# Daniel-Starr/pointcloudhookup

Measured on AMD Instinct MI355X. Metric: Mpts/s ground-filter+tower-cluster, 100 M-pt corridor; % HBM roofline on kNN, higher is better.
Workload: dtype f32 (filter) + f64 (distance predicate)

## Files before the change

pointcloudhookup_amd/csrc/pch_common.h:

```cpp
#pragma once
#include <hip/hip_runtime.h>
#include <stdint.h>
#include <stddef.h>
#include <stdio.h>
#include <string.h>

#include "../../include/pch_hip.h"

namespace pch {

void set_error(const char* fmt, ...);

#define PCH_HIP_TRY(expr)                                                         \
    do {                                                                          \
        hipError_t _e = (expr);                                                   \
        if (_e != hipSuccess) {                                                   \
            ::pch::set_error("%s failed: %s (%s:%d)", #expr, hipGetErrorString(_e), \
                             __FILE__, __LINE__);                                 \
            return PCH_ERR_HIP;                                                   \
        }                                                                         \
    } while (0)

#define PCH_TRY(expr)                  \
    do {                               \
        int _rc = (expr);              \
        if (_rc != PCH_OK) return _rc; \
    } while (0)

#define PCH_REQUIRE(cond, msg)                                   \
    do {                                                         \
        if (!(cond)) {                                           \
            ::pch::set_error("%s: %s", __func__, msg);           \
            return PCH_ERR_ARG;                                  \
        }                                                        \
    } while (0)

constexpr int PCH_MAX_DEVICES = 16;
struct DeviceGuard {
    int rc, prev, dev;
    explicit DeviceGuard(const void* device_ptr);
    ~DeviceGuard();
    DeviceGuard(const DeviceGuard&) = delete;
    DeviceGuard& operator=(const DeviceGuard&) = delete;
};
int current_device_slot();
bool may_release_hip_objects();
#define PCH_DEVICE_GUARD(ptr)                 \
    ::pch::DeviceGuard _pch_guard(ptr);       \
    if (_pch_guard.rc != PCH_OK) return _pch_guard.rc

void ws_touched(const void* base, size_t bytes);
struct Arena {
    char*  base;
    size_t cap;
    size_t off;
    bool   overflow;
    explicit Arena(void* b = nullptr, size_t c = 0, bool continues = false)
        : base(static_cast<char*>(b)), cap(c), off(0), overflow(false) {
        if (b && !continues) ws_touched(b, c);
    }
    template <typename T>
    T* take(size_t count) {
        size_t bytes = (count * sizeof(T) + 255) & ~size_t(255);
        size_t at = off;
        off += bytes;
        if (!base) return nullptr;
        if (off > cap) { overflow = true; return nullptr; }
        return reinterpret_cast<T*>(base + at);
    }
    size_t mark() const { return off; }
    void   reset(size_t m) { off = m; }
};

struct HostPeek {
    void*      pinned;
    hipEvent_t ev;
    bool       ok;
};
HostPeek& host_peek();
int peek_enqueue(const void* dev, size_t bytes, hipStream_t s);
int peek_wait(void* dst, size_t bytes);

struct DbBoxOut { uint32_t* acc; int32_t cap; bool done; };
struct GfEarly { const void* dev; size_t bytes; };
int ground_filter_run(const float* raw, int64_t n, double pct, float offset, float fallback_offset, int64_t min_keep,
                      float* out_points, int32_t* out_index, float* out_scalars, int64_t* out_count, float* out_aabb,
                      void* ws, size_t ws_bytes, hipStream_t s, const GfEarly* early);
int dbscan_run(const float* xyz, int64_t n, double eps, int32_t min_samples, int64_t chunk_size,
               const float* aabb_host, int32_t* labels, uint8_t* core, int32_t* out_nclusters,
               void* ws, size_t ws_bytes, hipStream_t s, int32_t* k_host, DbBoxOut* box = nullptr);
int segment_run(const int32_t* labels, const float* xyz, int64_t n, int32_t nclusters, int32_t* out_perm,
                int64_t* out_offsets, float* out_stats, void* ws, size_t ws_bytes, hipStream_t s, bool stats_encoded);

bool prof_enabled();
bool prof_wanted(const char* name);
void prof_pre(const char* name, hipStream_t s);
void prof_post(hipStream_t s);

#define PCH_LAUNCH(name, kernel, grid, block, shmem, stream, ...)                  \
    do {                                                                           \
        const bool _prof = ::pch::prof_enabled() && ::pch::prof_wanted(name);            \
        if (_prof) ::pch::prof_pre(name, stream);                                  \
        hipLaunchKernelGGL(kernel, grid, block, shmem, stream, __VA_ARGS__);       \
        if (_prof) ::pch::prof_post(stream);                                       \
        hipError_t _le = hipGetLastError();                                        \
        if (_le != hipSuccess) {                                                   \
            ::pch::set_error("launch %s failed: %s", name, hipGetErrorString(_le)); \
            return PCH_ERR_HIP;                                                    \
        }                                                                          \
    } while (0)

static inline int64_t ceil_div(int64_t a, int64_t b) { return (a + b - 1) / b; }
static inline int bits_for(uint64_t count) {
    int b = 0;
    while (b < 64 && (uint64_t(1) << b) < count) ++b;
    return b;
}

#ifdef __HIPCC__
constexpr int WAVE = 64;

__device__ __forceinline__ int lane_id() { return threadIdx.x & 63; }
__device__ __forceinline__ int wave_id() { return threadIdx.x >> 6; }

__device__ __forceinline__ uint32_t f32_ordered(float f) {
    uint32_t u = __float_as_uint(f);
    return (u & 0x80000000u) ? ~u : (u | 0x80000000u);
}
__device__ __forceinline__ float f32_unordered(uint32_t k) {
    uint32_t u = (k & 0x80000000u) ? (k & 0x7fffffffu) : ~k;
    return __uint_as_float(u);
}
__device__ __forceinline__ uint64_t f64_ordered(double d) {
    uint64_t u = (uint64_t)__double_as_longlong(d);
    return (u & 0x8000000000000000ull) ? ~u : (u | 0x8000000000000000ull);
}
__device__ __forceinline__ double f64_unordered(uint64_t k) {
    uint64_t u = (k & 0x8000000000000000ull) ? (k & 0x7fffffffffffffffull) : ~k;
    return __longlong_as_double((long long)u);
}

__device__ __forceinline__ uint64_t lanemask_lt() {
    return (uint64_t(1) << lane_id()) - 1;
}

template <typename T>
__device__ __forceinline__ T wave_reduce_add(T v) {
#pragma unroll
    for (int o = 32; o > 0; o >>= 1) v += __shfl_xor(v, o, 64);
    return v;
}
template <typename T>
__device__ __forceinline__ T wave_reduce_min(T v) {
#pragma unroll
    for (int o = 32; o > 0; o >>= 1) { T w = __shfl_xor(v, o, 64); v = w < v ? w : v; }
    return v;
}
template <typename T>
__device__ __forceinline__ T wave_reduce_max(T v) {
#pragma unroll
    for (int o = 32; o > 0; o >>= 1) { T w = __shfl_xor(v, o, 64); v = w > v ? w : v; }
    return v;
}
template <typename T>
__device__ __forceinline__ T wave_scan_incl(T v) {
    const int l = lane_id();
#pragma unroll
    for (int o = 1; o < 64; o <<= 1) { T w = __shfl_up(v, o, 64); if (l >= o) v += w; }
    return v;
}
template <int BITS>
__device__ __forceinline__ uint32_t wave_match(uint32_t d, bool valid, uint32_t& peers_out) {
    uint32_t nlo = 0, nhi = 0;
#pragma unroll
    for (int b = 0; b < BITS; ++b) {
        const int32_t B = ((int32_t)(d << (31 - b))) >> 31;
        const uint64_t m = __ballot(B != 0);
        nlo |= (uint32_t)m ^ (uint32_t)B;
        nhi |= (uint32_t)(m >> 32) ^ (uint32_t)B;
    }
    const uint64_t v = __ballot(valid);
    const uint32_t plo = (uint32_t)v & ~nlo, phi = (uint32_t)(v >> 32) & ~nhi;
    peers_out = (uint32_t)__popc(plo) + (uint32_t)__popc(phi);
    return __builtin_amdgcn_mbcnt_hi(phi, __builtin_amdgcn_mbcnt_lo(plo, 0u));
}
#endif

}
```

pointcloudhookup_amd/csrc/pch_dbscan.hip:

```cpp
#include "pch_prims.h"

namespace pch {

constexpr int DB_THREADS = 256;
constexpr int DB_WAVES   = DB_THREADS / 64;
constexpr int DB_ROWS    = 25;
constexpr int INT_BIG    = 0x7fffffff;
constexpr int DB_FEW_QUERIES = 24;
constexpr int DB_AHEAD = 3;
constexpr long long DB_LONG_TOT = 8192;
constexpr int DB_SEGS = 43;

struct DbGrid {
    float   ox, oy, oz;
    double  cell;
    double  inv_cell;
    double  eps2;
    float   eps2_lo, eps2_hi;
    int     bx, by, bz;
    int     mx, my, mz;
    int64_t chunk_size;
    const uint32_t* chunk_bad;
    const uint32_t* chunk_cells;
    int     min_samples;
};

__constant__ int8_t DB_ROW_DY[DB_ROWS] = {0, 1, -1, 0, 0, 1, 1, -1, -1, 2, -2, 0, 0,
                                          2, 2, -2, -2, 1, 1, -1, -1, 2, 2, -2, -2};
__constant__ int8_t DB_ROW_DZ[DB_ROWS] = {0, 0, 0, 1, -1, 1, -1, 1, -1, 0, 0, 2, -2,
                                          1, -1, 1, -1, 2, -2, 2, -2, 2, -2, 2, -2};

__device__ __forceinline__ uint64_t db_pack(const DbGrid& g, uint64_t chunk, uint64_t cz,
                                            uint64_t cy, uint64_t cx) {
    return ((((chunk << g.bz) | cz) << g.by | cy) << g.bx) | cx;
}

__device__ __forceinline__ bool db_within(const float4& q, const float4& p, double eps2) {
    const double dx = (double)q.x - (double)p.x;
    const double dy = (double)q.y - (double)p.y;
    const double dz = (double)q.z - (double)p.z;
    double d = dx * dx;
    d += dy * dy;
    d += dz * dz;
    return d <= eps2;
}

__device__ __forceinline__ bool db_within2(const float4& q, const float4& p, const DbGrid& g) {
    const float dx = q.x - p.x, dy = q.y - p.y, dz = q.z - p.z;
    float d = dx * dx;
    d = __builtin_fmaf(dy, dy, d);
    d = __builtin_fmaf(dz, dz, d);
    if (d <= g.eps2_lo) return true;
    if (d >= g.eps2_hi) return false;
    return db_within(q, p, g.eps2);
}

typedef float f32x2 __attribute__((ext_vector_type(2)));
struct __attribute__((aligned(16))) DbPair { f32x2 x, y, z, pad; };

__device__ __forceinline__ void db_tile_put(DbPair* __restrict__ tile, int l, const float4& p) {
    float* f = reinterpret_cast<float*>(&tile[l >> 1]);
    f[l & 1] = p.x; f[2 + (l & 1)] = p.y; f[4 + (l & 1)] = p.z;
}
__device__ __forceinline__ float4 db_tile_get(const DbPair* __restrict__ tile, int k) {
    const float* f = reinterpret_cast<const float*>(&tile[k >> 1]);
    float4 p;
    p.x = f[k & 1]; p.y = f[2 + (k & 1)]; p.z = f[4 + (k & 1)]; p.w = 0.0f;
    return p;
}
__device__ __forceinline__ int db_tile_count(const float4& q, const DbPair* __restrict__ tile, int nj,
                                             const DbGrid& g) {
    const f32x2 qx = {q.x, q.x}, qy = {q.y, q.y}, qz = {q.z, q.z};
    const float lo = g.eps2_lo, hi = g.eps2_hi;
    int c_lo = 0, c_hi = 0;
    const int np = ((nj + 7) & ~7) >> 1;
    for (int k = 0; k < np; k += 4) {
        f32x2 px[4], py[4], pz[4];
#pragma unroll
        for (int u = 0; u < 4; ++u) { px[u] = tile[k + u].x; py[u] = tile[k + u].y; pz[u] = tile[k + u].z; }
#pragma unroll
        for (int u = 0; u < 4; ++u) {
            const f32x2 dx = qx - px[u], dy = qy - py[u], dz = qz - pz[u];
            f32x2 d = dx * dx;
            d = __builtin_elementwise_fma(dy, dy, d);
            d = __builtin_elementwise_fma(dz, dz, d);
            c_lo += (d.x <= lo ? 1 : 0) + (d.y <= lo ? 1 : 0);
            c_hi += (d.x < hi ? 1 : 0) + (d.y < hi ? 1 : 0);
        }
    }
    if (c_lo != c_hi) {
        c_lo = 0;
        for (int k = 0; k < nj; ++k) c_lo += db_within2(q, db_tile_get(tile, k), g) ? 1 : 0;
    }
    return c_lo;
}

__device__ __forceinline__ double db_box_d2(const float4& q, const float* __restrict__ box) {
    const double gx = fmax(fmax((double)box[0] - (double)q.x, (double)q.x - (double)box[3]), 0.0);
    const double gy = fmax(fmax((double)box[1] - (double)q.y, (double)q.y - (double)box[4]), 0.0);
    const double gz = fmax(fmax((double)box[2] - (double)q.z, (double)q.z - (double)box[5]), 0.0);
    double d = gx * gx;
    d += gy * gy;
    d += gz * gz;
    return d;
}
__device__ __forceinline__ double db_boxbox_d2(const float* __restrict__ a, const float* __restrict__ b) {
    const double gx = fmax(fmax((double)b[0] - (double)a[3], (double)a[0] - (double)b[3]), 0.0);
    const double gy = fmax(fmax((double)b[1] - (double)a[4], (double)a[1] - (double)b[4]), 0.0);
    const double gz = fmax(fmax((double)b[2] - (double)a[5], (double)a[2] - (double)b[5]), 0.0);
    double d = gx * gx;
    d += gy * gy;
    d += gz * gz;
    return d;
}

__device__ __forceinline__ bool db_row_bad(const float* __restrict__ xyz, int64_t i) {
    const uint32_t a = __float_as_uint(xyz[3 * i + 0]) & 0x7FFFFFFFu;
    const uint32_t b = __float_as_uint(xyz[3 * i + 1]) & 0x7FFFFFFFu;
    const uint32_t c = __float_as_uint(xyz[3 * i + 2]) & 0x7FFFFFFFu;
    return a >= 0x7F800000u || b >= 0x7F800000u || c >= 0x7F800000u;
}
__global__ __launch_bounds__(DB_THREADS) void db_chunkbad_k(const float* __restrict__ xyz, int64_t n,
                                                            int64_t chunk_size, uint32_t* __restrict__ bad) {
    for (int64_t i = (int64_t)blockIdx.x * DB_THREADS + threadIdx.x; i < n;
         i += (int64_t)gridDim.x * DB_THREADS)
        if (db_row_bad(xyz, i)) atomicOr(&bad[i / chunk_size], 1u);
}

__global__ __launch_bounds__(DB_THREADS) void db_first_bad_k(const float* __restrict__ xyz, int64_t n,
                                                             unsigned long long* __restrict__ first) {
    unsigned long long best = ~0ull;
    for (int64_t i = (int64_t)blockIdx.x * DB_THREADS + threadIdx.x; i < n;
         i += (int64_t)gridDim.x * DB_THREADS)
        if (db_row_bad(xyz, i) && (unsigned long long)i < best) best = (unsigned long long)i;
    best = wave_reduce_min(best);
    if (lane_id() == 0 && best != ~0ull) atomicMin(first, best);
}

__global__ __launch_bounds__(DB_THREADS) void db_aabb_in_k(const float* __restrict__ xyz, int64_t n,
                                                           uint32_t* __restrict__ mm) {
    uint32_t lo[3] = {0xFFFFFFFFu, 0xFFFFFFFFu, 0xFFFFFFFFu}, hi[3] = {0u, 0u, 0u};
    for (int64_t i = (int64_t)blockIdx.x * DB_THREADS + threadIdx.x; i < n;
         i += (int64_t)gridDim.x * DB_THREADS) {
        const float x = xyz[3 * i + 0], y = xyz[3 * i + 1], z = xyz[3 * i + 2];
        if (!(fabsf(x) < INFINITY && fabsf(y) < INFINITY && fabsf(z) < INFINITY)) continue;
        const float v[3] = {x, y, z};
#pragma unroll
        for (int a = 0; a < 3; ++a) {
            const uint32_t k = f32_ordered(v[a]);
            lo[a] = k < lo[a] ? k : lo[a];
            hi[a] = k > hi[a] ? k : hi[a];
        }
    }
#pragma unroll
    for (int a = 0; a < 3; ++a) {
        lo[a] = wave_reduce_min(lo[a]);
        hi[a] = wave_reduce_max(hi[a]);
        if (lane_id() == 0) {
            if (lo[a] != 0xFFFFFFFFu) atomicMin(&mm[a], lo[a]);
            if (hi[a] != 0u) atomicMax(&mm[3 + a], hi[a]);
        }
    }
}

__device__ __forceinline__ bool db_cell_coords(const DbGrid& g, float x, float y, float z,
                                               uint32_t& cx, uint32_t& cy, uint32_t& cz) {
    const double fx = floor(((double)x - (double)g.ox) * g.inv_cell);
    const double fy = floor(((double)y - (double)g.oy) * g.inv_cell);
    const double fz = floor(((double)z - (double)g.oz) * g.inv_cell);
    const bool ok = fx >= 0.0 && fx <= (double)g.mx && fy >= 0.0 && fy <= (double)g.my &&
                    fz >= 0.0 && fz <= (double)g.mz;
    cx = ok ? (uint32_t)fx : 0u; cy = ok ? (uint32_t)fy : 0u; cz = ok ? (uint32_t)fz : 0u;
    return ok;
}

__global__ __launch_bounds__(DB_THREADS) void db_keys_k(const float* __restrict__ xyz, int64_t n,
                                                        DbGrid g, const uint32_t* __restrict__ bad,
                                                        uint64_t* __restrict__ keys,
                                                        uint32_t* __restrict__ vals,
                                                        uint32_t* __restrict__ status) {
    const int64_t i = (int64_t)blockIdx.x * DB_THREADS + threadIdx.x;
    if (i >= n) return;
    vals[i] = (uint32_t)i;
    if (bad[i / g.chunk_size]) {
        keys[i] = db_pack(g, (uint64_t)(i / g.chunk_size), 0, 0, 0);
        return;
    }
    const float x = xyz[3 * i + 0], y = xyz[3 * i + 1], z = xyz[3 * i + 2];
    uint32_t cx, cy, cz;
    if (!db_cell_coords(g, x, y, z, cx, cy, cz)) atomicOr(status, 1u);
    keys[i] = db_pack(g, (uint64_t)(i / g.chunk_size), cz, cy, cx);
}

__global__ __launch_bounds__(DB_THREADS) void dbc_axis_keys_k(const float* __restrict__ xyz, int64_t n, int axis,
                                                              uint64_t* __restrict__ keys, uint32_t* __restrict__ vals) {
    const int64_t i = (int64_t)blockIdx.x * DB_THREADS + threadIdx.x;
    if (i >= n) return;
    keys[i] = f32_ordered(xyz[3 * i + axis]);
    vals[i] = (uint32_t)i;
}
__global__ __launch_bounds__(DB_THREADS) void dbc_heads_k(const uint64_t* __restrict__ keys, int64_t n, double inv_cell,
                                                          uint32_t* __restrict__ head) {
    const int64_t i = (int64_t)blockIdx.x * DB_THREADS + threadIdx.x;
    if (i >= n) return;
    bool h = i == 0;
    if (i > 0) {
        const double a = (double)f32_unordered((uint32_t)keys[i - 1]), b = (double)f32_unordered((uint32_t)keys[i]);
        h = (b - a) * inv_cell >= 3.0;
    }
    head[i] = h ? 1u : 0u;
}
__global__ __launch_bounds__(DB_THREADS) void dbc_local_k(const uint64_t* __restrict__ keys, const uint32_t* __restrict__ flag,
                                                          const uint32_t* __restrict__ excl, int64_t n, double inv_cell,
                                                          float* __restrict__ headx, int phase,
                                                          uint32_t* __restrict__ li, uint32_t* __restrict__ seglen,
                                                          uint32_t* __restrict__ status) {
    const int64_t i = (int64_t)blockIdx.x * DB_THREADS + threadIdx.x;
    if (i >= n) return;
    const uint32_t seg = excl[i] + flag[i] - 1u;
    const float x = f32_unordered((uint32_t)keys[i]);
    if (phase == 0) {
        if (flag[i]) headx[seg] = x;
        return;
    }
    const double v = floor(((double)x - (double)headx[seg]) * inv_cell);
    uint32_t u = 0;
    if (v >= 0.0 && v < 2147483000.0) u = (uint32_t)v; else atomicOr(status, 2u);
    li[i] = u;
    const bool last = i + 1 == n || flag[i + 1] != 0u;
    if (last) seglen[seg] = u + 3u;
}
__global__ __launch_bounds__(DB_THREADS) void dbc_comp_k(const uint32_t* __restrict__ vals, const uint32_t* __restrict__ flag,
                                                         const uint32_t* __restrict__ excl, const uint32_t* __restrict__ li,
                                                         const uint32_t* __restrict__ segoff, int64_t n, int axis,
                                                         uint32_t* __restrict__ comp, uint32_t* __restrict__ cmax) {
    const int64_t i = (int64_t)blockIdx.x * DB_THREADS + threadIdx.x;
    if (i >= n) return;
    const uint32_t seg = excl[i] + flag[i] - 1u;
    const uint32_t c = segoff[seg] + li[i];
    comp[3 * (int64_t)vals[i] + axis] = c;
    if (i == n - 1) cmax[axis] = c;
}
__global__ __launch_bounds__(DB_THREADS) void db_keys_comp_k(const uint32_t* __restrict__ comp, int64_t n, DbGrid g,
                                                             uint64_t* __restrict__ keys, uint32_t* __restrict__ vals) {
    const int64_t i = (int64_t)blockIdx.x * DB_THREADS + threadIdx.x;
    if (i >= n) return;
    vals[i] = (uint32_t)i;
    keys[i] = db_pack(g, 0, comp[3 * i + 2], comp[3 * i + 1], comp[3 * i + 0]);
}
__global__ __launch_bounds__(DB_THREADS) void db_add_offset_k(int32_t* __restrict__ labels, int64_t n, int32_t off) {
    const int64_t i = (int64_t)blockIdx.x * DB_THREADS + threadIdx.x;
    if (i < n && labels[i] >= 0) labels[i] += off;
}

__global__ __launch_bounds__(DB_THREADS) void db_gather_k(const float* __restrict__ xyz,
                                                          const uint64_t* __restrict__ keys,
                                                          const uint32_t* __restrict__ vals, int64_t n,
                                                          float4* __restrict__ pts) {
    const int64_t i = (int64_t)blockIdx.x * DB_THREADS + threadIdx.x;
    if (i >= n) return;
    const uint32_t o = vals[i];
    float4 p;
    p.x = xyz[3 * (int64_t)o + 0];
    p.y = xyz[3 * (int64_t)o + 1];
    p.z = xyz[3 * (int64_t)o + 2];
    p.w = __uint_as_float(o);
    pts[i] = p;
}

struct Row3 { float x, y, z; };
constexpr int CS_THREADS = 1024;
constexpr int CS_WAVES   = CS_THREADS / 64;
constexpr int CS_ROUNDS  = 4;
constexpr int CS_TILE    = CS_THREADS * CS_ROUNDS;
constexpr int CS_PASSES  = 4;
constexpr int CS_HREP    = 4;
constexpr int CS_BINS    = 512;
constexpr int64_t CS_MAX_CHUNK = 1 << 17;
constexpr int64_t CS_MIN_CHUNKS = 96;

__device__ __forceinline__ uint32_t cs_cell_key(const DbGrid& g, float x, float y, float z, bool& ok) {
    uint32_t cx, cy, cz;
    ok = db_cell_coords(g, x, y, z, cx, cy, cz);
    return (((cz << g.by) | cy) << g.bx) | cx;
}

__global__ __launch_bounds__(CS_THREADS) void db_chunksort_k(
    const float* __restrict__ xyz, int64_t n, DbGrid g, const uint32_t* __restrict__ gate, uint32_t* __restrict__ bad,
    float4* __restrict__ xbuf, float4* __restrict__ pts, uint64_t* __restrict__ keys_out,
    uint32_t* __restrict__ status, unsigned long long* __restrict__ stamps) {
    if (gate[blockIdx.x] == 0u) return;
#ifdef PCH_CS_STAMPS
    int stamp_i = 0;
#define CS_STAMP() if (stamps && blockIdx.x == gridDim.x / 2 && threadIdx.x == 0) stamps[stamp_i++] = wall_clock64();
    unsigned long long tacc[3] = {0, 0, 0}, tlast = 0;
#define CS_TILE_STAMP(k) do { const unsigned long long _t = wall_clock64(); tacc[k] += _t - tlast; tlast = _t; } while (0)
#else
#define CS_STAMP()
#define CS_TILE_STAMP(k)
#endif
    CS_STAMP();
    __shared__ uint32_t hist[CS_PASSES][CS_HREP][CS_BINS];
    __shared__ uint32_t cnt[CS_WAVES][CS_BINS];
    __shared__ uint32_t off[CS_WAVES][CS_BINS];
    __shared__ uint32_t base[CS_BINS];
    __shared__ uint32_t wsum[CS_BINS / 64];
    __shared__ uint32_t flags[2];
    __shared__ uint32_t cbox[6];
    const int tid = threadIdx.x, w = wave_id(), l = lane_id();
    const int64_t c = blockIdx.x;
    const int64_t lo = c * g.chunk_size;
    const int cn = (int)((n - lo) < g.chunk_size ? (n - lo) : g.chunk_size);
    const Row3* __restrict__ rows = reinterpret_cast<const Row3*>(xyz) + lo;
    for (int j = tid; j < CS_PASSES * CS_HREP * CS_BINS; j += CS_THREADS) (&hist[0][0][0])[j] = 0;
    for (int j = tid; j < CS_WAVES * CS_BINS; j += CS_THREADS) (&cnt[0][0])[j] = 0;
    if (tid < 2) flags[tid] = 0;
    if (tid < 6) cbox[tid] = tid < 3 ? 0xFFFFFFFFu : 0u;
    __syncthreads();
    constexpr int HU = 8;
    {
        uint32_t mn[3] = {0xFFFFFFFFu, 0xFFFFFFFFu, 0xFFFFFFFFu}, mx[3] = {0u, 0u, 0u};
        for (int i0 = 0; i0 < cn; i0 += HU * CS_THREADS) {
            Row3 q[HU];
#pragma unroll
            for (int u = 0; u < HU; ++u) {
                const int i = i0 + u * CS_THREADS + tid;
                q[u] = rows[i < cn ? i : 0];
            }
#pragma unroll
            for (int u = 0; u < HU; ++u) {
                const bool in = i0 + u * CS_THREADS + tid < cn;
                const bool fin = fabsf(q[u].x) < INFINITY && fabsf(q[u].y) < INFINITY && fabsf(q[u].z) < INFINITY;
                uint32_t cc[3];
                const bool ok = db_cell_coords(g, q[u].x, q[u].y, q[u].z, cc[0], cc[1], cc[2]);
                if (in && !fin) flags[0] = 1u;
                else if (in && !ok) flags[1] = 1u;
                if (in && fin && ok) {
#pragma unroll
                    for (int a = 0; a < 3; ++a) { mn[a] = cc[a] < mn[a] ? cc[a] : mn[a]; mx[a] = cc[a] > mx[a] ? cc[a] : mx[a]; }
                }
            }
        }
#pragma unroll
        for (int a = 0; a < 3; ++a) {
            const uint32_t lo_w = wave_reduce_min(mn[a]), hi_w = wave_reduce_max(mx[a]);
            if (l == 0) { atomicMin(&cbox[a], lo_w); atomicMax(&cbox[3 + a], hi_w); }
        }
    }
    __syncthreads();
    CS_STAMP();
    const uint32_t ox = cbox[0], oy = cbox[1], oz = cbox[2];
    const bool any = cbox[3] >= ox && cbox[4] >= oy && cbox[5] >= oz;
    const int wx = any && cbox[3] > ox ? 32 - __clz(cbox[3] - ox) : 0;
    const int wy = any && cbox[4] > oy ? 32 - __clz(cbox[4] - oy) : 0;
    const int wz = any && cbox[5] > oz ? 32 - __clz(cbox[5] - oz) : 0;
    const int tb = wx + wy + wz;
    const int passes = (tb + 8) / 9;
    const int dbits = passes ? (tb + passes - 1) / passes : 1;
    const uint32_t mask = (1u << dbits) - 1u;
    const uint32_t gxm = (1u << g.bx) - 1u, gym = (1u << g.by) - 1u;
    auto relkey = [&](uint32_t k) -> uint32_t {
        const uint32_t cx = k & gxm, cy = (k >> g.bx) & gym, cz = k >> (g.bx + g.by);
        return (uint32_t)((((((uint64_t)(cz - oz)) << wy) | (uint64_t)(cy - oy)) << wx) | (uint64_t)(cx - ox));
    };
    for (int i0 = 0; i0 < cn; i0 += HU * CS_THREADS) {
        Row3 q[HU];
#pragma unroll
        for (int u = 0; u < HU; ++u) {
            const int i = i0 + u * CS_THREADS + tid;
            q[u] = rows[i < cn ? i : 0];
        }
#pragma unroll
        for (int u = 0; u < HU; ++u) {
            const bool in = i0 + u * CS_THREADS + tid < cn;
            bool ok;
            const uint32_t k = relkey(cs_cell_key(g, q[u].x, q[u].y, q[u].z, ok));
            if (in)
                for (int p = 0; p < passes; ++p) atomicAdd(&hist[p][l & (CS_HREP - 1)][(k >> (p * dbits)) & mask], 1u);
        }
    }
    __syncthreads();
    const bool isbad = flags[0] != 0;
    CS_STAMP();
    if (tid == 0) {
        bad[c] = isbad ? 1u : 0u;
        if (!isbad && flags[1]) atomicOr(status, 1u);
    }
    const int sh = g.bx + g.by + g.bz;
    const uint64_t hi = sh < 64 ? ((uint64_t)c << sh) : 0ull;
    if (isbad || passes == 0) {
        for (int i = tid; i < cn; i += CS_THREADS) {
            const Row3 q = rows[i];
            float4 o4;
            o4.x = q.x; o4.y = q.y; o4.z = q.z; o4.w = __uint_as_float((uint32_t)(lo + i));
            pts[lo + i] = o4;
            bool ok;
            keys_out[lo + i] = isbad ? hi : (hi | cs_cell_key(g, q.x, q.y, q.z, ok));
        }
        return;
    }
    auto run_pass = [&](int p, auto FIRST_T, auto LAST_T) {
        constexpr bool FIRST = decltype(FIRST_T)::value, LAST = decltype(LAST_T)::value;
        const int shift = p * dbits;
        const float4* __restrict__ src = ((passes - p) & 1) ? xbuf + lo : pts + lo;
        float4* __restrict__ dst = ((passes - 1 - p) & 1) ? xbuf + lo : pts + lo;
        uint32_t hv = 0, incl = 0;
        if (tid < CS_BINS) {
            hv = 0;
#pragma unroll
            for (int r = 0; r < CS_HREP; ++r) hv += hist[p][r][tid];
            incl = wave_scan_incl(hv);
            if (l == 63) wsum[w] = incl;
        }
        __syncthreads();
        if (tid < CS_BINS) {
            uint32_t b = incl - hv;
            for (int w2 = 0; w2 < w; ++w2) b += wsum[w2];
            base[tid] = b;
        }
        __syncthreads();
        auto fetch = [&](int t0, float4 (&out)[CS_ROUNDS]) {
            const int seg = t0 + w * (64 * CS_ROUNDS);
#pragma unroll
            for (int r = 0; r < CS_ROUNDS; ++r) {
                const int i = seg + r * 64 + l;
                const int j = i < cn ? i : 0;
                if constexpr (FIRST) {
                    const Row3 q = rows[j];
                    out[r].x = q.x; out[r].y = q.y; out[r].z = q.z;
                    out[r].w = __uint_as_float((uint32_t)(lo + j));
                } else {
                    out[r] = src[j];
                }
            }
        };
        float4 nxt[CS_ROUNDS];
        auto tile = [&](int t0, auto FULL_T) {
            constexpr bool FULL = decltype(FULL_T)::value;
            float4 row[CS_ROUNDS];
            uint32_t key[CS_ROUNDS], rank[CS_ROUNDS];
            const int seg = t0 + w * (64 * CS_ROUNDS);
#pragma unroll
            for (int r = 0; r < CS_ROUNDS; ++r) row[r] = nxt[r];
            if (t0 + CS_TILE < cn) fetch(t0 + CS_TILE, nxt);
#ifdef PCH_CS_STAMPS
            tlast = wall_clock64();
#endif
#pragma unroll
            for (int r = 0; r < CS_ROUNDS; ++r) {
                const bool valid = FULL || seg + r * 64 + l < cn;
                bool ok;
                key[r] = cs_cell_key(g, row[r].x, row[r].y, row[r].z, ok);
                const uint32_t d = (relkey(key[r]) >> shift) & mask;
                uint32_t np;
                const uint32_t rk = dbits <= 8 ? wave_match<8>(d, valid, np) : wave_match<9>(d, valid, np);
                const uint32_t prior = cnt[w][d];
                __builtin_amdgcn_wave_barrier();
                if (valid && rk == 0) cnt[w][d] = prior + np;
                __builtin_amdgcn_wave_barrier();
                rank[r] = prior + rk;
            }
            __syncthreads();
            CS_TILE_STAMP(0);
            if (tid < CS_BINS) {
                uint32_t run = base[tid];
#pragma unroll
                for (int w2 = 0; w2 < CS_WAVES; ++w2) {
                    const uint32_t cc = cnt[w2][tid];
                    off[w2][tid] = run;
                    cnt[w2][tid] = 0;
                    run += cc;
                }
                base[tid] = run;
            }
            __syncthreads();
            CS_TILE_STAMP(1);
#pragma unroll
            for (int r = 0; r < CS_ROUNDS; ++r) {
                if (FULL || seg + r * 64 + l < cn) {
                    const uint32_t d = (relkey(key[r]) >> shift) & mask;
                    const uint32_t pos = off[w][d] + rank[r];
                    dst[pos] = row[r];
                    if constexpr (LAST) keys_out[lo + pos] = hi | key[r];
                }
            }
            CS_TILE_STAMP(2);
        };
        fetch(0, nxt);
        int t0 = 0;
        for (; t0 + CS_TILE <= cn; t0 += CS_TILE) tile(t0, std::true_type{});
        if (t0 < cn) tile(t0, std::false_type{});
        __syncthreads();
        CS_STAMP();
    };
    for (int p = 0; p < passes; ++p) {
        const bool first = p == 0, last = p == passes - 1;
        if (first && last) run_pass(p, std::true_type{}, std::true_type{});
        else if (first)    run_pass(p, std::true_type{}, std::false_type{});
        else if (last)     run_pass(p, std::false_type{}, std::true_type{});
        else               run_pass(p, std::false_type{}, std::false_type{});
    }
#ifdef PCH_CS_STAMPS
    __syncthreads();
    CS_STAMP();
    if (stamps && blockIdx.x == gridDim.x / 2 && threadIdx.x == 0) for (int k = 0; k < 3; ++k) stamps[8 + k] = tacc[k];
#endif
}

constexpr int CT_SLOTS = 4096;
constexpr int CT_BITS  = 12;
constexpr int CT_CELLS = 1024;
constexpr uint32_t CT_EMPTY = 0xFFFFFFFFu;
static_assert(CT_SLOTS == 1 << CT_BITS && CT_CELLS + CS_THREADS < CT_SLOTS, "the table never fills (see sweep 1)");

__device__ __forceinline__ uint32_t ct_hash(uint32_t k) { return (k * 0x9E3779B1u) >> (32 - CT_BITS); }

__global__ __launch_bounds__(CS_THREADS) void db_cellscatter_k(
    const float* __restrict__ xyz, int64_t n, DbGrid g, uint32_t* __restrict__ bad, uint32_t* __restrict__ ovf,
    float4* __restrict__ pts, uint64_t* __restrict__ keys_out, uint32_t* __restrict__ status) {
    __shared__ uint32_t tkey[CT_SLOTS];
    __shared__ uint32_t tcnt[CT_SLOTS];
    __shared__ uint32_t skey[CT_CELLS];
    __shared__ uint32_t wsum[CS_WAVES];
    __shared__ uint32_t flags[5];
    const int tid = threadIdx.x, w = wave_id(), l = lane_id();
    const int64_t c = blockIdx.x;
    const int64_t lo = c * g.chunk_size;
    const int cn = (int)((n - lo) < g.chunk_size ? (n - lo) : g.chunk_size);
    const Row3* __restrict__ rows = reinterpret_cast<const Row3*>(xyz) + lo;
    for (int j = tid; j < CT_SLOTS; j += CS_THREADS) { tkey[j] = CT_EMPTY; tcnt[j] = 0u; }
    if (tid < 5) flags[tid] = 0u;
    __syncthreads();
    constexpr int HU = 8;
    for (int i0 = 0; i0 < cn; i0 += HU * CS_THREADS) {
        if (__hip_atomic_load(&flags[3], __ATOMIC_RELAXED, __HIP_MEMORY_SCOPE_WORKGROUP)) break;
        Row3 q[HU];
#pragma unroll
        for (int u = 0; u < HU; ++u) {
            const int i = i0 + u * CS_THREADS + tid;
            q[u] = rows[i < cn ? i : 0];
        }
#pragma unroll
        for (int u = 0; u < HU; ++u) {
            const bool in = i0 + u * CS_THREADS + tid < cn;
            const bool fin = fabsf(q[u].x) < INFINITY && fabsf(q[u].y) < INFINITY && fabsf(q[u].z) < INFINITY;
            bool ok;
            const uint32_t k = cs_cell_key(g, q[u].x, q[u].y, q[u].z, ok);
            if (in && !fin) flags[0] = 1u;
            else if (in && !ok) flags[1] = 1u;
            if (in && fin && __hip_atomic_load(&flags[3], __ATOMIC_RELAXED, __HIP_MEMORY_SCOPE_WORKGROUP) == 0u) {
                uint32_t h = ct_hash(k);
                for (int p = 0; p < CT_SLOTS; ++p, h = (h + 1u) & (CT_SLOTS - 1)) {
                    const uint32_t old = atomicCAS(&tkey[h], CT_EMPTY, k);
                    if (old == CT_EMPTY && atomicAdd(&flags[2], 1u) >= (uint32_t)CT_CELLS) flags[3] = 1u;
                    if (old == CT_EMPTY || old == k) { atomicAdd(&tcnt[h], 1u); break; }
                }
            }
        }
    }
    __syncthreads();
    const bool isbad = flags[0] != 0u;
    const uint32_t ncell = flags[2];
    const bool over = !isbad && ncell > (uint32_t)CT_CELLS;
    if (tid == 0) {
        ovf[c] = over ? 1u : 0u;
        if (!over) {
            bad[c] = isbad ? 1u : 0u;
            if (!isbad && flags[1]) atomicOr(status, 1u);
        }
    }
    if (over) return;
    const int sh = g.bx + g.by + g.bz;
    const uint64_t hi = sh < 64 ? ((uint64_t)c << sh) : 0ull;
    if (isbad || ncell == 1u) {
        for (int i = tid; i < cn; i += CS_THREADS) {
            const Row3 q = rows[i];
            float4 o4;
            o4.x = q.x; o4.y = q.y; o4.z = q.z; o4.w = __uint_as_float((uint32_t)(lo + i));
            pts[lo + i] = o4;
            bool ok;
            keys_out[lo + i] = isbad ? hi : (hi | cs_cell_key(g, q.x, q.y, q.z, ok));
        }
        return;
    }
    const int P = 1 << (32 - __clz((int)ncell - 1));
    for (int j0 = 0; j0 < CT_SLOTS; j0 += CS_THREADS) {
        const uint32_t k = tkey[j0 + tid];
        const uint64_t m = __ballot(k != CT_EMPTY);
        uint32_t base = 0;
        if (l == 0 && m) base = atomicAdd(&flags[4], (uint32_t)__popcll(m));
        base = (uint32_t)__shfl((int)base, 0, 64);
        if (k != CT_EMPTY) skey[base + (uint32_t)__popcll(m & lanemask_lt())] = k;
    }
    for (int j = (int)ncell + tid; j < P; j += CS_THREADS) skey[j] = CT_EMPTY;
    __syncthreads();
    for (int k = 2; k <= P; k <<= 1) {
        for (int j = k >> 1; j > 0; j >>= 1) {
            for (int t = tid; t < P / 2; t += CS_THREADS) {
                const int a = 2 * t - (t & (j - 1)), b = a + j;
                const uint32_t ka = skey[a], kb = skey[b];
                if ((ka > kb) == ((a & k) == 0)) { skey[a] = kb; skey[b] = ka; }
            }
            __syncthreads();
        }
    }
    {
        uint32_t slot[4], cnt[4], sum = 0;
#pragma unroll
        for (int u = 0; u < 4; ++u) {
            const int j = 4 * tid + u;
            slot[u] = 0; cnt[u] = 0;
            if (j < (int)ncell) {
                const uint32_t k = skey[j];
                uint32_t h = ct_hash(k);
                for (int p = 0; p < CT_SLOTS && tkey[h] != k; ++p) h = (h + 1u) & (CT_SLOTS - 1);
                slot[u] = h;
                cnt[u] = tcnt[h];
            }
            sum += cnt[u];
        }
        const uint32_t incl = wave_scan_incl(sum);
        if (l == 63) wsum[w] = incl;
        __syncthreads();
        uint32_t run = incl - sum;
        for (int w2 = 0; w2 < w; ++w2) run += wsum[w2];
#pragma unroll
        for (int u = 0; u < 4; ++u) {
            if (4 * tid + u < (int)ncell) tcnt[slot[u]] = run;
            run += cnt[u];
        }
    }
    __syncthreads();
    for (int i0 = 0; i0 < cn; i0 += HU * CS_THREADS) {
        Row3 q[HU];
#pragma unroll
        for (int u = 0; u < HU; ++u) {
            const int i = i0 + u * CS_THREADS + tid;
            q[u] = rows[i < cn ? i : 0];
        }
#pragma unroll
        for (int u = 0; u < HU; ++u) {
            const int i = i0 + u * CS_THREADS + tid;
            if (i < cn) {
                bool ok;
                const uint32_t k = cs_cell_key(g, q[u].x, q[u].y, q[u].z, ok);
                uint32_t h = ct_hash(k);
                for (int p = 0; p < CT_SLOTS && tkey[h] != k; ++p) h = (h + 1u) & (CT_SLOTS - 1);
                const uint32_t pos = atomicAdd(&tcnt[h], 1u);
                if (pos >= (uint32_t)cn) continue;
                float4 o4;
                o4.x = q[u].x; o4.y = q[u].y; o4.z = q[u].z; o4.w = __uint_as_float((uint32_t)(lo + i));
                pts[lo + pos] = o4;
                keys_out[lo + pos] = hi | k;
            }
        }
    }
}

constexpr int DC_ITEMS = SCAN_TILE / DB_THREADS;
static_assert(DC_ITEMS == 8, "two 64-byte key loads per thread");

__device__ __forceinline__ void dc_load_keys(const uint64_t* __restrict__ keys, int64_t base, int64_t n,
                                             uint64_t (&k)[DC_ITEMS], uint64_t& prev) {
    if (base + DC_ITEMS <= n) {
        const ulonglong2* q = reinterpret_cast<const ulonglong2*>(keys + base);
#pragma unroll
        for (int j = 0; j < DC_ITEMS / 2; ++j) { const ulonglong2 v = q[j]; k[2 * j] = v.x; k[2 * j + 1] = v.y; }
    } else {
#pragma unroll
        for (int j = 0; j < DC_ITEMS; ++j) k[j] = base + j < n ? keys[base + j] : 0ull;
    }
    prev = (base > 0 && base < n) ? keys[base - 1] : 0ull;
}

__global__ __launch_bounds__(DB_THREADS) void db_heads_k(const uint64_t* __restrict__ keys, int64_t n,
                                                         uint32_t* __restrict__ tile_sums) {
    __shared__ uint32_t wsum[DB_WAVES];
    const int64_t base = (int64_t)blockIdx.x * SCAN_TILE + (int64_t)threadIdx.x * DC_ITEMS;
    uint64_t k[DC_ITEMS], prev;
    dc_load_keys(keys, base, n, k, prev);
    uint32_t heads = 0;
#pragma unroll
    for (int j = 0; j < DC_ITEMS; ++j) {
        const int64_t i = base + j;
        heads += (i < n && (i == 0 || k[j] != (j ? k[j - 1] : prev))) ? 1u : 0u;
    }
    heads = wave_reduce_add(heads);
    if (lane_id() == 0) wsum[wave_id()] = heads;
    __syncthreads();
    if (threadIdx.x == 0) {
        uint32_t t = 0;
#pragma unroll
        for (int w = 0; w < DB_WAVES; ++w) t += wsum[w];
        tile_sums[blockIdx.x] = t;
    }
}

__global__ __launch_bounds__(DB_THREADS) void db_cells_k(const uint64_t* __restrict__ keys,
                                                         const uint32_t* __restrict__ tile_excl, int64_t n,
                                                         int sh, int64_t nchunks,
                                                         uint32_t* __restrict__ cid,
                                                         uint32_t* __restrict__ cell_start,
                                                         uint64_t* __restrict__ cell_key,
                                                         uint32_t* __restrict__ chunk_cells,
                                                         uint32_t* __restrict__ cell_acc) {
    __shared__ uint32_t wsum[DB_WAVES];
    const int64_t base = (int64_t)blockIdx.x * SCAN_TILE + (int64_t)threadIdx.x * DC_ITEMS;
    uint64_t k[DC_ITEMS], prev;
    dc_load_keys(keys, base, n, k, prev);
    bool hd[DC_ITEMS];
    uint32_t heads = 0;
#pragma unroll
    for (int j = 0; j < DC_ITEMS; ++j) {
        const int64_t i = base + j;
        hd[j] = i < n && (i == 0 || k[j] != (j ? k[j - 1] : prev));
        heads += hd[j] ? 1u : 0u;
    }
    const uint32_t incl = wave_scan_incl(heads);
    if (lane_id() == 63) wsum[wave_id()] = incl;
    __syncthreads();
    uint32_t c = tile_excl[blockIdx.x] + incl - heads;
    for (int w = 0; w < wave_id(); ++w) c += wsum[w];
    uint32_t cc[DC_ITEMS];
#pragma unroll
    for (int j = 0; j < DC_ITEMS; ++j) {
        const int64_t i = base + j;
        c += hd[j] ? 1u : 0u;
        cc[j] = c - 1u;
        if (hd[j]) {
            const uint64_t key = k[j], pk = j ? k[j - 1] : prev;
            cell_start[cc[j]] = (uint32_t)i;
            cell_key[cc[j]] = key;
            uint4* a4 = reinterpret_cast<uint4*>(cell_acc + 8 * (int64_t)cc[j]);
            a4[0] = make_uint4(0u, 0u, 0u, 0u);
            a4[1] = make_uint4(0u, 0u, 0u, 0u);
            const uint64_t ch = sh < 64 ? key >> sh : 0, pch = sh < 64 ? pk >> sh : 0;
            if (i == 0 || ch != pch) chunk_cells[ch] = cc[j];
        }
        if (i == n - 1) { cell_start[cc[j] + 1] = (uint32_t)n; chunk_cells[nchunks] = cc[j] + 1; }
    }
    if (base + DC_ITEMS <= n) {
        uint4* o = reinterpret_cast<uint4*>(cid + base);
        o[0] = make_uint4(cc[0], cc[1], cc[2], cc[3]);
        o[1] = make_uint4(cc[4], cc[5], cc[6], cc[7]);
    } else {
#pragma unroll
        for (int j = 0; j < DC_ITEMS; ++j)
            if (base + j < n) cid[base + j] = cc[j];
    }
}
struct RowSet {
    int ca[DB_ROWS], cb[DB_ROWS];
};

__device__ __forceinline__ int db_lower(const uint64_t* __restrict__ a, int m, uint64_t k) {
    int lo = 0, hi = m;
    while (lo < hi) { const int mid = (lo + hi) >> 1; if (a[mid] < k) lo = mid + 1; else hi = mid; }
    return lo;
}
__device__ __forceinline__ int2 db_row_run(const DbGrid& g, const uint64_t* __restrict__ cell_key, uint64_t key,
                                           int row) {
    const uint64_t cx = key & ((1ull << g.bx) - 1);
    const uint64_t cy = (key >> g.bx) & ((1ull << g.by) - 1);
    const uint64_t cz = (key >> (g.bx + g.by)) & ((1ull << g.bz) - 1);
    const int sh = g.bx + g.by + g.bz;
    const uint64_t chunk = sh < 64 ? (key >> sh) : 0;
    const int ny = (int)cy + DB_ROW_DY[row], nz = (int)cz + DB_ROW_DZ[row];
    int2 v;
    v.x = 0; v.y = 0;
    if (ny >= 0 && ny <= g.my && nz >= 0 && nz <= g.mz) {
        const int xlo = (int)cx - 2 < 0 ? 0 : (int)cx - 2;
        const int xhi = (int)cx + 2 > g.mx ? g.mx : (int)cx + 2;
        const int c0 = (int)g.chunk_cells[chunk], c1 = (int)g.chunk_cells[chunk + 1];
        v.x = c0 + db_lower(cell_key + c0, c1 - c0, db_pack(g, chunk, (uint64_t)nz, (uint64_t)ny, (uint64_t)xlo));
        const uint64_t khi = db_pack(g, chunk, (uint64_t)nz, (uint64_t)ny, (uint64_t)xhi);
        uint64_t kk[5];
#pragma unroll
        for (int i = 0; i < 5; ++i) kk[i] = v.x + i < c1 ? cell_key[v.x + i] : ~0ull;
        int cntx = 0;
#pragma unroll
        for (int i = 0; i < 5; ++i) cntx += kk[i] <= khi ? 1 : 0;
        v.y = v.x + cntx;
    }
    return v;
}

__device__ __forceinline__ void db_rows(const DbGrid& g, const uint64_t* __restrict__ cell_key, uint64_t key,
                                        RowSet* __restrict__ rs, const int2* __restrict__ rowtab, int cell) {
    const int l = lane_id();
    if (rowtab) {
        if (l < DB_ROWS) {
            const int2 v = rowtab[(int64_t)cell * DB_ROWS + l];
            rs->ca[l] = v.x;
            rs->cb[l] = v.y;
        }
        __builtin_amdgcn_wave_barrier();
        return;
    }
    if (l < DB_ROWS) {
        const int2 v = db_row_run(g, cell_key, key, l);
        rs->ca[l] = v.x;
        rs->cb[l] = v.y;
    }
    __builtin_amdgcn_wave_barrier();
}

__global__ __launch_bounds__(DB_THREADS) void db_rowtab_k(DbGrid g, const uint64_t* __restrict__ cell_key,
                                                          int m, int2* __restrict__ rowtab) {
    const int c = (blockIdx.x * DB_WAVES + wave_id()) * 2 + (lane_id() >> 5);
    const int l = lane_id() & 31;
    if (c >= m || l >= DB_ROWS) return;
    rowtab[(int64_t)c * DB_ROWS + l] = db_row_run(g, cell_key, cell_key[c], l);
}

template <bool COUNT>
__global__ __launch_bounds__(DB_THREADS) void db_core_k(DbGrid g, const float4* __restrict__ pts,
                                                        const uint32_t* __restrict__ cell_start,
                                                        const uint64_t* __restrict__ cell_key, int m,
                                                        const int2* __restrict__ rowtab,
                                                        uint8_t* __restrict__ core_s,
                                                        uint32_t* __restrict__ cell_ncore,
                                                        unsigned long long* __restrict__ stats) {
    unsigned long long n_useful = 0, n_slots = 0, n_tiles = 0;
    auto tally = [&]() {
        if (COUNT && lane_id() == 0) {
            atomicAdd(&stats[0], n_useful); atomicAdd(&stats[1], n_slots);
            atomicAdd(&stats[2], 1ull); atomicAdd(&stats[3], n_tiles);
        }
    };
    __shared__ RowSet rows[DB_WAVES];
    __shared__ DbPair tiles[DB_WAVES][32];
    __shared__ uint32_t seg_a[DB_WAVES][DB_SEGS], seg_b[DB_WAVES][DB_SEGS];
    const int c = blockIdx.x * DB_WAVES + wave_id();
    if (c >= m) return;
    const int l = lane_id();
    const uint32_t s = cell_start[c], e = cell_start[c + 1];
    const int cnt = (int)(e - s);
    {
        const int sh = g.bx + g.by + g.bz;
        if (g.chunk_bad[sh < 64 ? (cell_key[c] >> sh) : 0]) {
            for (uint32_t i = s + l; i < e; i += 64) core_s[i] = 0;
            if (l == 0) cell_ncore[c] = 0;
            return;
        }
    }
    if (cnt >= g.min_samples) {
        for (uint32_t i = s + l; i < e; i += 64) core_s[i] = 1;
        if (l == 0) cell_ncore[c] = (uint32_t)cnt;
        return;
    }
    RowSet* rs = &rows[wave_id()];
    db_rows(g, cell_key, cell_key[c], rs, rowtab, c);
    long long tot = 0;
    if (l < DB_ROWS) tot = (long long)cell_start[rs->cb[l]] - (long long)cell_start[rs->ca[l]];
    tot = wave_reduce_add(tot);
    if (tot < (long long)g.min_samples) {
        for (uint32_t i = s + l; i < e; i += 64) core_s[i] = 0;
        if (l == 0) cell_ncore[c] = 0;
        return;
    }
    uint32_t* sa = seg_a[wave_id()];
    uint32_t* sb = seg_b[wave_id()];
    {
        const uint64_t xmask = (1ull << g.bx) - 1;
        const int cx = (int)(cell_key[c] & xmask);
        if (l < DB_ROWS) {
            const int ca = rs->ca[l], cb = rs->cb[l];
            if (l < 9) {
                int ia = ca, ib = cb;
                if (ca < cb) {
                    if ((int)(cell_key[ca] & xmask) == cx - 2) ia = ca + 1;
                    if (ib > ia && (int)(cell_key[cb - 1] & xmask) == cx + 2) ib = cb - 1;
                }
                sa[l] = cell_start[ia];      sb[l] = cell_start[ib];
                sa[9 + l] = cell_start[ca];  sb[9 + l] = cell_start[ia];
                sa[18 + l] = cell_start[ib]; sb[18 + l] = cell_start[cb];
            } else {
                sa[18 + l] = cell_start[ca]; sb[18 + l] = cell_start[cb];
            }
        }
        __builtin_amdgcn_wave_barrier();
    }
    uint32_t ncore = 0;
    const bool long_sweep = tot >= DB_LONG_TOT;
    if (cnt < DB_FEW_QUERIES) {
        for (uint32_t q = s; q < e; ++q) {
            const float4 qp = pts[q];
            int count = 0;
            if (long_sweep) {
                for (int r = 0; r < DB_SEGS && count < g.min_samples; ++r) {
                    const uint32_t pa = sa[r], pb = sb[r];
                    for (uint32_t j0 = pa; j0 < pb && count < g.min_samples; j0 += 64u * DB_AHEAD) {
                        float4 P[DB_AHEAD];
#pragma unroll
                        for (int u = 0; u < DB_AHEAD; ++u) {
                            const uint32_t j = j0 + 64u * u + l;
                            P[u] = pts[j < pb ? j : pb - 1];
                        }
#pragma unroll
                        for (int u = 0; u < DB_AHEAD; ++u) {
                            const uint32_t jb = j0 + 64u * u;
                            const bool hit = jb + l < pb && db_within2(qp, P[u], g);
                            count += (int)__popcll(__ballot(hit));
                            if (COUNT && jb < pb) { n_useful += (pb - jb) < 64u ? (pb - jb) : 64u; n_slots += 64; }
                        }
                    }
                }
            } else {
                for (int r = 0; r < DB_SEGS && count < g.min_samples; ++r) {
                    const uint32_t pa = sa[r], pb = sb[r];
                    for (uint32_t j0 = pa; j0 < pb && count < g.min_samples; j0 += 64) {
                        const uint32_t j = j0 + l;
                        bool hit = false;
                        if (j < pb) hit = db_within2(qp, pts[j], g);
                        count += (int)__popcll(__ballot(hit));
                        if (COUNT) { n_useful += (pb - j0) < 64u ? (pb - j0) : 64u; n_slots += 64; }
                    }
                }
            }
            const bool is_core = count >= g.min_samples;
            if (l == 0) core_s[q] = is_core ? 1 : 0;
            ncore += is_core;
        }
        if (l == 0) cell_ncore[c] = ncore;
        tally();
        return;
    }
    DbPair* tile = tiles[wave_id()];
    for (uint32_t q0 = s; q0 < e; q0 += 64) {
        const bool valid = q0 + l < e;
        float4 Q;
        Q.x = Q.y = Q.z = 3.0e37f; Q.w = 0.0f;
        if (valid) Q = pts[q0 + l];
        int count = 0;
        unsigned long long active = __ballot(valid);
        int r = 0;
        uint32_t j0 = sa[0];
        while (r < DB_SEGS && __popcll(active) >= DB_FEW_QUERIES / 2) {
            const uint32_t pb = sb[r];
            if (j0 >= pb) { ++r; if (r < DB_SEGS) j0 = sa[r]; continue; }
            const int nj = (int)((pb - j0) < 64u ? (pb - j0) : 64u);
            float4 P;
            P.x = P.y = P.z = 3.0e38f; P.w = 0.0f;
            if (l < nj) P = pts[j0 + l];
            __builtin_amdgcn_wave_barrier();
            db_tile_put(tile, l, P);
            __builtin_amdgcn_wave_barrier();
            count += db_tile_count(Q, tile, nj, g);
            if (COUNT) {
                n_useful += (unsigned long long)__popcll(__ballot(valid)) * (unsigned)nj;
                n_slots += 64ull * (unsigned)((nj + 7) & ~7);
                ++n_tiles;
            }
            j0 += 64;
            active = __ballot(valid && count < g.min_samples);
        }
        while (active) {
            const int ql = (int)__builtin_ctzll(active);
            active &= active - 1;
            float4 qp;
            qp.x = __shfl(Q.x, ql, 64); qp.y = __shfl(Q.y, ql, 64); qp.z = __shfl(Q.z, ql, 64); qp.w = 0.0f;
            int cq = __shfl(count, ql, 64);
            int rr = r;
            uint32_t jj = j0;
            if (long_sweep) {
                while (rr < DB_SEGS && cq < g.min_samples) {
                    const uint32_t pb = sb[rr];
                    if (jj >= pb) { ++rr; if (rr < DB_SEGS) jj = sa[rr]; continue; }
                    float4 P[DB_AHEAD];
#pragma unroll
                    for (int u = 0; u < DB_AHEAD; ++u) {
                        const uint32_t j = jj + 64u * u + l;
                        P[u] = pts[j < pb ? j : pb - 1];
                    }
#pragma unroll
                    for (int u = 0; u < DB_AHEAD; ++u) {
                        const uint32_t jb = jj + 64u * u;
                        const bool hit = jb + l < pb && db_within2(qp, P[u], g);
                        cq += (int)__popcll(__ballot(hit));
                        if (COUNT && jb < pb) { n_useful += (pb - jb) < 64u ? (pb - jb) : 64u; n_slots += 64; }
                    }
                    jj += 64u * DB_AHEAD;
                }
            } else {
                while (rr < DB_SEGS && cq < g.min_samples) {
                    const uint32_t pb = sb[rr];
                    if (jj >= pb) { ++rr; if (rr < DB_SEGS) jj = sa[rr]; continue; }
                    const uint32_t j = jj + l;
                    bool hit = false;
                    if (j < pb) hit = db_within2(qp, pts[j], g);
                    cq += (int)__popcll(__ballot(hit));
                    if (COUNT) { n_useful += (pb - jj) < 64u ? (pb - jj) : 64u; n_slots += 64; }
                    jj += 64;
                }
            }
            if (l == ql) count = cq;
        }
        const bool is_core = valid && count >= g.min_samples;
        if (valid) core_s[q0 + l] = is_core ? 1 : 0;
        ncore += (uint32_t)__popcll(__ballot(is_core));
    }
    if (l == 0) cell_ncore[c] = ncore;
    tally();
}

constexpr int DB_CS_ROUNDS = 16;

__device__ __forceinline__ void db_cellstats_flush(uint32_t* __restrict__ acc, uint32_t c, const uint32_t (&v)[7]) {
#pragma unroll
    for (int k = 0; k < 7; ++k)
        if (v[k]) atomicMax(&acc[8 * (int64_t)c + k], v[k]);
}

__global__ __launch_bounds__(DB_THREADS) void db_cellstats_k(const float4* __restrict__ pts,
                                                             const uint32_t* __restrict__ cid,
                                                             const uint8_t* __restrict__ core_s, int64_t n,
                                                             uint32_t* __restrict__ acc,
                                                             uint32_t* __restrict__ bits, int64_t nw) {
    {
        const int64_t t = (int64_t)blockIdx.x * DB_THREADS + threadIdx.x;
        if (t < nw) bits[t] = 0u;
    }
    const int64_t base = ((int64_t)blockIdx.x * DB_WAVES + wave_id()) * (64 * DB_CS_ROUNDS);
    if (base >= n) return;
    const int l = lane_id();
    constexpr uint32_t NONE = 0xFFFFFFFFu;
    uint32_t carry_c = NONE;
    uint32_t carry[7] = {0, 0, 0, 0, 0, 0, 0};
    uint32_t mine[7] = {0, 0, 0, 0, 0, 0, 0};
    auto fold_mine = [&]() {
#pragma unroll
        for (int k = 0; k < 7; ++k) {
            const uint32_t t = wave_reduce_max(mine[k]);
            carry[k] = t > carry[k] ? t : carry[k];
            mine[k] = 0;
        }
    };
    for (int r0 = 0; r0 < DB_CS_ROUNDS; r0 += 4) {
    if (base + r0 * 64 >= n) break;
    uint32_t c4[4], core4[4];
    float4 p4[4];
#pragma unroll
    for (int u = 0; u < 4; ++u) {
        const int64_t i = base + (r0 + u) * 64 + l;
        const bool in = i < n;
        c4[u] = in ? cid[i] : NONE - 1u;
        core4[u] = in ? core_s[i] : 0u;
        p4[u] = pts[in ? i : base];
    }
#pragma unroll
    for (int u = 0; u < 4; ++u) {
        const int64_t i = base + (r0 + u) * 64 + l;
        const bool in = i < n;
        const uint32_t c = c4[u];
        uint32_t v[7] = {0, 0, 0, 0, 0, 0, 0};
        if (core4[u]) {
            const float4 p = p4[u];
            const uint32_t kx = f32_ordered(p.x), ky = f32_ordered(p.y), kz = f32_ordered(p.z);
            v[0] = ~kx; v[1] = ~ky; v[2] = ~kz; v[3] = kx; v[4] = ky; v[5] = kz;
            v[6] = ~__float_as_uint(p.w);
        }
        if (__ballot(c != carry_c) == 0) {
#pragma unroll
            for (int k = 0; k < 7; ++k) mine[k] = v[k] > mine[k] ? v[k] : mine[k];
            continue;
        }
        if (carry_c != NONE) fold_mine();
#pragma unroll
        for (int o = 1; o < 64; o <<= 1) {
            const uint32_t cu = __shfl_up(c, o, 64);
            const bool same = l >= o && cu == c;
#pragma unroll
            for (int k = 0; k < 7; ++k) {
                const uint32_t t = __shfl_up(v[k], o, 64);
                if (same) v[k] = t > v[k] ? t : v[k];
            }
        }
        const uint32_t c0 = (uint32_t)__builtin_amdgcn_readlane((int)c, 0);
        if (carry_c != NONE) {
            if (carry_c == c0) {
                if (c == c0) {
#pragma unroll
                    for (int k = 0; k < 7; ++k) v[k] = carry[k] > v[k] ? carry[k] : v[k];
                }
            } else if (l == 0) {
                db_cellstats_flush(acc, carry_c, carry);
            }
        }
        const uint32_t cn = __shfl_down(c, 1, 64);
        const bool run_end = l == 63 || cn != c;
        if (run_end && l != 63 && in) db_cellstats_flush(acc, c, v);
        carry_c = (uint32_t)__builtin_amdgcn_readlane((int)c, 63);
        if (carry_c == NONE - 1u) carry_c = NONE;
#pragma unroll
        for (int k = 0; k < 7; ++k) carry[k] = (uint32_t)__builtin_amdgcn_readlane((int)v[k], 63);
    }
    }
    if (carry_c != NONE) {
        fold_mine();
        if (l == 0) db_cellstats_flush(acc, carry_c, carry);
    }
}

__global__ __launch_bounds__(DB_THREADS) void db_cellfin_k(const uint32_t* __restrict__ acc, int m,
                                                           float* __restrict__ cell_box,
                                                           int* __restrict__ cell_min,
                                                           int* __restrict__ parent,
                                                           int* __restrict__ comp_min) {
    const int c = blockIdx.x * DB_THREADS + threadIdx.x;
    if (c >= m) return;
    uint32_t a[7];
#pragma unroll
    for (int k = 0; k < 7; ++k) a[k] = acc[8 * (int64_t)c + k];
    float box[6];
#pragma unroll
    for (int k = 0; k < 3; ++k) {
        box[k] = INFINITY;
        box[3 + k] = -INFINITY;
        if (a[k] != 0u) box[k] = f32_unordered(~a[k]);
        if (a[3 + k] != 0u) box[3 + k] = f32_unordered(a[3 + k]);
    }
#pragma unroll
    for (int k = 0; k < 6; ++k) cell_box[6 * (int64_t)c + k] = box[k];
    int mn = INT_BIG;
    if (a[6] != 0u) mn = (int)(~a[6]);
    cell_min[c] = mn;
    parent[c] = c;
    comp_min[c] = INT_BIG;
}

__device__ __forceinline__ float db_d2f(const float4& a, const float4& b) {
    const float dx = a.x - b.x, dy = a.y - b.y, dz = a.z - b.z;
    return __builtin_fmaf(dz, dz, __builtin_fmaf(dy, dy, dx * dx));
}
__device__ __forceinline__ float db_box_d2f(const float4& q, const float* __restrict__ box) {
    const float gx = fmaxf(fmaxf(box[0] - q.x, q.x - box[3]), 0.0f);
    const float gy = fmaxf(fmaxf(box[1] - q.y, q.y - box[4]), 0.0f);
    const float gz = fmaxf(fmaxf(box[2] - q.z, q.z - box[5]), 0.0f);
    return __builtin_fmaf(gz, gz, __builtin_fmaf(gy, gy, gx * gx));
}
template <typename F>
__device__ __forceinline__ int db_argmin(const float4* __restrict__ pts, const uint8_t* __restrict__ core_s,
                                         uint32_t s, uint32_t e, bool dense, F f) {
    const int l = lane_id();
    unsigned long long best = ~0ull;
    for (uint32_t i0 = s; i0 < e; i0 += 256) {
#pragma unroll
        for (int u = 0; u < 4; ++u) {
            const uint32_t i = i0 + 64 * u + l;
            if (i < e && (dense || core_s[i])) {
                const float d = f(pts[i]);
                const unsigned long long k = ((unsigned long long)__float_as_uint(d) << 32) | i;
                best = k < best ? k : best;
            }
        }
    }
    best = wave_reduce_min(best);
    return best == ~0ull ? -1 : (int)(uint32_t)best;
}

__device__ __forceinline__ bool db_cells_connected(const DbGrid& g, const float4* __restrict__ pts,
                                                   const uint8_t* __restrict__ core_s, uint32_t as, uint32_t ae,
                                                   bool a_dense, uint32_t bs, uint32_t be, bool b_dense,
                                                   const float* __restrict__ boxB, uint32_t a_from) {
    const int l = lane_id();
    if (ae - as > 64 || be - bs > 64) {
        int ia = db_argmin(pts, core_s, as, ae, a_dense, [&](const float4& p) { return db_box_d2f(p, boxB); });
        if (ia < 0) return false;
        float4 q = pts[ia];
        for (int it = 0; it < 3; ++it) {
            const int jb = db_argmin(pts, core_s, bs, be, b_dense, [&](const float4& p) { return db_d2f(q, p); });
            if (jb < 0) return false;
            const float4 pb = pts[jb];
            if (db_within2(q, pb, g)) return true;
            const int ia2 = db_argmin(pts, core_s, as, ae, a_dense, [&](const float4& p) { return db_d2f(p, pb); });
            const float4 pa = pts[ia2];
            if (db_within2(pa, pb, g)) return true;
            if (ia2 == ia) break;
            ia = ia2;
            q = pa;
        }
    }
    for (uint32_t a0 = a_from; a0 < ae; a0 += 64) {
        const uint32_t ia = a0 + l;
        float4 pa;
        pa.x = pa.y = pa.z = pa.w = 0.0f;
        bool near = false;
        if (ia < ae && (a_dense || core_s[ia])) {
            pa = pts[ia];
            near = !(db_box_d2(pa, boxB) > g.eps2);
        }
        unsigned long long todo = __ballot(near);
        while (todo) {
            const int src = (int)__builtin_ctzll(todo);
            todo &= todo - 1;
            float4 q;
            q.x = __shfl(pa.x, src, 64); q.y = __shfl(pa.y, src, 64); q.z = __shfl(pa.z, src, 64); q.w = 0.0f;
            for (uint32_t j0 = bs; j0 < be; j0 += 64) {
                const uint32_t j = j0 + l;
                bool hit = false;
                if (j < be && (b_dense || core_s[j])) hit = db_within2(q, pts[j], g);
                if (__ballot(hit)) return true;
            }
        }
    }
    return false;
}

__device__ __forceinline__ int uf_load(int* p) {
    return __hip_atomic_load(p, __ATOMIC_RELAXED, __HIP_MEMORY_SCOPE_AGENT);
}
__device__ __forceinline__ int uf_find(int* __restrict__ parent, int x) {
    int p = uf_load(&parent[x]);
    while (p != x) {
        const int gp = uf_load(&parent[p]);
        if (gp != p) __hip_atomic_store(&parent[x], gp, __ATOMIC_RELAXED, __HIP_MEMORY_SCOPE_AGENT);
        x = p;
        p = gp;
    }
    return x;
}
__device__ __forceinline__ void uf_union(int* __restrict__ parent, int a, int b) {
    for (;;) {
        a = uf_find(parent, a);
        b = uf_find(parent, b);
        if (a == b) return;
        if (a < b) { const int t = a; a = b; b = t; }
        const int old = atomicCAS(&parent[a], a, b);
        if (old == a) return;
        a = old;
    }
}

struct DbFace { int row; uint64_t want; };
__device__ __forceinline__ DbFace db_face(const DbGrid& g, uint64_t key, int dir) {
    return {dir == 1 ? 1 : 3, key + (dir == 0 ? 1ull : (dir == 1 ? (1ull << g.bx) : (1ull << (g.bx + g.by))))};
}
__device__ __forceinline__ bool db_link_open(const DbGrid& g, const float* __restrict__ cell_box,
                                             const float* __restrict__ boxB, const int* parent, int A, int B) {
    return !(db_boxbox_d2(cell_box + 6 * (int64_t)A, boxB) > g.eps2) && parent[A] != parent[B];
}

__global__ __launch_bounds__(DB_THREADS) void db_union_k(DbGrid g, const float4* __restrict__ pts,
                                                         const uint32_t* __restrict__ cell_start,
                                                         const uint64_t* __restrict__ cell_key, int m,
                                                         const int2* __restrict__ rowtab,
                                                         const uint8_t* __restrict__ core_s,
                                                         const uint32_t* __restrict__ cell_ncore,
                                                         const float* __restrict__ cell_box,
                                                         int* __restrict__ parent) {
    __shared__ RowSet rows[DB_WAVES];
    __shared__ int cand[DB_WAVES][128];
    const int A = blockIdx.x * DB_WAVES + wave_id();
    if (A >= m) return;
    if (cell_ncore[A] == 0) return;
    const int l = lane_id();
    RowSet* rs = &rows[wave_id()];
    int* cd = cand[wave_id()];
    const uint64_t keyA = cell_key[A];
    db_rows(g, cell_key, keyA, rs, rowtab, A);
    int total;
    {
        int len = 0;
        if (l < DB_ROWS) { len = rs->cb[l] - rs->ca[l]; len = len < 0 ? 0 : len; }
        const int incl = wave_scan_incl(len);
        total = __shfl(incl, 63, 64);
        if (l < DB_ROWS)
            for (int k = 0; k < len; ++k) cd[incl - len + k] = rs->ca[l] + k;
    }
    __builtin_amdgcn_wave_barrier();
    const uint32_t as = cell_start[A], ae = cell_start[A + 1];
    const bool a_dense = cell_ncore[A] == (ae - as);
    for (int base = 0; base < total; base += 64) {
        int B = -1;
        if (base + l < total) B = cd[base + l];
        bool live = false;
        if (B > A) {
            live = cell_ncore[B] != 0 && db_link_open(g, cell_box, cell_box + 6 * (int64_t)B, parent, A, B);
            if (live) live = uf_find(parent, A) != uf_find(parent, B);
        }
        unsigned long long todo = __ballot(live);
        while (todo) {
            const int src = (int)__builtin_ctzll(todo);
            todo &= todo - 1;
            const int Bs = __builtin_amdgcn_readlane(B, src);
            {
                int same = 0;
                if (l == 0) same = uf_find(parent, A) == uf_find(parent, Bs);
                if (__builtin_amdgcn_readfirstlane(same)) continue;
            }
            const uint32_t bs = cell_start[Bs], be = cell_start[Bs + 1];
            const bool b_dense = cell_ncore[Bs] == (be - bs);
            const float* boxB = cell_box + 6 * (int64_t)Bs;
            const bool connected = db_cells_connected(g, pts, core_s, as, ae, a_dense, bs, be, b_dense, boxB, as);
            if (connected && l == 0) uf_union(parent, A, Bs);
        }
    }
}

constexpr int DB_PAIR_TRIES = 3;

__global__ __launch_bounds__(DB_THREADS) void db_union_pairs_k(DbGrid g, const float4* __restrict__ pts,
                                                               const uint32_t* __restrict__ cell_start,
                                                               const uint64_t* __restrict__ cell_key, int m,
                                                               const int2* __restrict__ rowtab,
                                                               const uint8_t* __restrict__ core_s,
                                                               const uint32_t* __restrict__ cell_ncore,
                                                               const float* __restrict__ cell_box,
                                                               int* __restrict__ parent,
                                                               uint8_t* __restrict__ face_todo) {
    const int64_t t = (int64_t)blockIdx.x * DB_THREADS + threadIdx.x;
    const int A = (int)(t >> 2), dir = (int)(t & 3);
    const bool lane_on = A < m && dir < 3;
    bool undecided = false;
    if (lane_on) {
        const uint32_t ncoreA = cell_ncore[A];
        if (ncoreA != 0) {
            const DbFace f = db_face(g, cell_key[A], dir);
            int B = -1;
            if (dir == 0) {
                if (A + 1 < m && cell_key[A + 1] == f.want) B = A + 1;
            } else {
                const int2 run = rowtab[(int64_t)A * DB_ROWS + f.row];
                for (int k = run.x; k < run.y; ++k)
                    if (cell_key[k] == f.want) { B = k; break; }
            }
            if (B > A) {
                const uint32_t nB = cell_ncore[B];
                if (nB != 0) {
                    float boxB[6];
#pragma unroll
                    for (int a = 0; a < 6; ++a) boxB[a] = cell_box[6 * (int64_t)B + a];
                    bool pend = db_link_open(g, cell_box, boxB, parent, A, B);
                    int rootA = A, rootB = B;
                    if (pend) {
                        rootA = uf_find(parent, A);
                        rootB = uf_find(parent, B);
                        pend = rootA != rootB;
                    }
                    if (pend) {
                        const uint32_t as = cell_start[A], ae = cell_start[A + 1];
                        const uint32_t bs = cell_start[B], be = cell_start[B + 1];
                        const bool a_dense = ncoreA == (ae - as), b_dense = nB == (be - bs);
                        float4 pb[DB_PAIR_TRIES];
                        int nb = 0;
                        for (uint32_t j = bs; j < be && nb < DB_PAIR_TRIES; ++j)
                            if (b_dense || core_s[j]) pb[nb++] = pts[j];
                        bool connected = false;
                        int na = 0;
                        for (uint32_t i = as; i < ae && na < DB_PAIR_TRIES && !connected; ++i) {
                            if (!a_dense && !core_s[i]) continue;
                            ++na;
                            const float4 pa = pts[i];
                            if (db_box_d2(pa, boxB) > g.eps2) continue;
#pragma unroll
                            for (int j = 0; j < DB_PAIR_TRIES; ++j)
                                if (j < nb && db_within2(pa, pb[j], g)) connected = true;
                        }
                        if (connected) uf_union(parent, rootA, rootB);
                        else undecided = true;
                    }
                }
            }
        }
    }
    const unsigned long long um = __ballot(undecided);
    if (A < m && dir == 0) face_todo[A] = (uint8_t)((um >> (lane_id() & ~3)) & 7ull);
}

constexpr int DB_FACE_TRIES = 8;

__global__ __launch_bounds__(DB_THREADS) void db_union_face_k(DbGrid g, const float4* __restrict__ pts,
                                                              const uint32_t* __restrict__ cell_start,
                                                              const uint64_t* __restrict__ cell_key, int m,
                                                              const int2* __restrict__ rowtab,
                                                              const uint8_t* __restrict__ core_s,
                                                              const uint32_t* __restrict__ cell_ncore,
                                                              const float* __restrict__ cell_box,
                                                              int* __restrict__ parent,
                                                              const uint8_t* __restrict__ face_todo) {
    __shared__ RowSet rows[DB_WAVES];
    const int A = blockIdx.x * DB_WAVES + wave_id();
    if (A >= m) return;
    if (face_todo && face_todo[A] == 0) return;
    const uint32_t ncoreA = cell_ncore[A];
    if (ncoreA == 0) return;
    const int l = lane_id();
    const int grp = l / 21, gl = l - 21 * grp;
    const unsigned long long gmask = grp < 3 ? (0x1FFFFFull << (21 * grp)) : 0ull;
    RowSet* rs = &rows[wave_id()];
    const uint64_t keyA = cell_key[A];
    db_rows(g, cell_key, keyA, rs, rowtab, A);
    int B = -1;
    {
        bool found = false;
        int k = -1;
        if (grp < 3) {
            const DbFace f = db_face(g, keyA, grp);
            if (grp == 0) {
                k = A + 1;
                found = gl == 0 && k < m && cell_key[k] == f.want;
            } else {
                k = rs->ca[f.row] + gl;
                found = k < rs->cb[f.row] && cell_key[k] == f.want;
            }
        }
        const unsigned long long fm = __ballot(found) & gmask;
        if (fm) B = __shfl(k, (int)__builtin_ctzll(fm), 64);
    }
    const uint32_t as = cell_start[A], ae = cell_start[A + 1];
    const bool a_dense = ncoreA == (ae - as);
    const float4 pa0 = pts[as];
    uint32_t bs = 0, be = 0;
    bool b_dense = false, pend = false;
    float boxB[6] = {0, 0, 0, 0, 0, 0};
    if (B > A) {
        const uint32_t nB = cell_ncore[B];
        bs = cell_start[B];
        be = cell_start[B + 1];
        b_dense = nB == (be - bs);
#pragma unroll
        for (int a = 0; a < 6; ++a) boxB[a] = cell_box[6 * (int64_t)B + a];
        pend = nB != 0 && db_link_open(g, cell_box, boxB, parent, A, B);
    }
    if (gl != 0) pend = false;
    int rootA = A, rootB = B;
    if (pend) {
        rootA = uf_find(parent, A);
        rootB = uf_find(parent, B);
        pend = rootA != rootB;
    }
    pend = __shfl((int)pend, grp < 3 ? 21 * grp : 0, 64) != 0 && grp < 3;
    bool connected = false;
    uint32_t ia = as;
    for (int tries = 0; ia < ae && tries < DB_FACE_TRIES; ++ia) {
        if (__ballot(pend) == 0) break;
        if (!a_dense && !core_s[ia]) continue;
        ++tries;
        const float4 pa = ia == as ? pa0 : pts[ia];
        bool near = pend && !(db_box_d2(pa, boxB) > g.eps2);
        const uint32_t maxlen = wave_reduce_max(near ? be - bs : 0u);
        for (uint32_t j0 = 0; j0 < maxlen; j0 += 21) {
            const uint32_t j = bs + j0 + gl;
            bool hit = false;
            if (near && j < be && (b_dense || core_s[j])) hit = db_within2(pa, pts[j], g);
            if (__ballot(hit) & gmask) { connected = true; pend = false; near = false; }
            if (__ballot(near) == 0) break;
        }
    }
    if (connected && gl == 0) uf_union(parent, rootA, rootB);
    unsigned long long todo = __ballot(pend && gl == 0);
    while (todo) {
        const int src = (int)__builtin_ctzll(todo);
        todo &= todo - 1;
        const int Bs = __shfl(B, src, 64);
        const uint32_t bs2 = cell_start[Bs], be2 = cell_start[Bs + 1];
        const bool b_dense2 = cell_ncore[Bs] == (be2 - bs2);
        const float* boxB2 = cell_box + 6 * (int64_t)Bs;
        const bool conn = db_cells_connected(g, pts, core_s, as, ae, a_dense, bs2, be2, b_dense2, boxB2, ia);
        if (conn && l == 0) uf_union(parent, A, Bs);
    }
}

__global__ __launch_bounds__(DB_THREADS) void db_flatten_k(int* __restrict__ parent, int m) {
    const int c = blockIdx.x * DB_THREADS + threadIdx.x;
    if (c >= m) return;
    const int r = uf_find(parent, c);
    if (r != c) parent[c] = r;
}

__global__ __launch_bounds__(DB_THREADS) void db_compmin_k(const int* __restrict__ cell_min,
                                                           const uint32_t* __restrict__ cell_ncore, int m,
                                                           int* __restrict__ parent,
                                                           int* __restrict__ root,
                                                           int* __restrict__ comp_min) {
    const int c = blockIdx.x * DB_THREADS + threadIdx.x;
    if (c >= m) return;
    if (cell_ncore[c] == 0) { root[c] = -1; return; }
    const int r = uf_find(parent, c);
    root[c] = r;
    atomicMin(&comp_min[r], cell_min[c]);
}

__global__ __launch_bounds__(DB_THREADS) void db_mark_k(const int* __restrict__ root,
                                                        const int* __restrict__ comp_min, int m,
                                                        uint32_t* __restrict__ flag) {
    const int c = blockIdx.x * DB_THREADS + threadIdx.x;
    if (c >= m) return;
    if (root[c] == c) {
        const uint32_t r = (uint32_t)comp_min[c];
        atomicOr(&flag[r >> 5], 1u << (r & 31u));
    }
}

constexpr int DB_LAB_ROUNDS = 8;
constexpr int DB_LAB_TILE   = DB_THREADS * DB_LAB_ROUNDS;

__device__ __forceinline__ void db_box_flush(uint32_t* __restrict__ acc, int cur, uint32_t (&m)[6]) {
    const int l = lane_id();
    uint32_t v = 0;
#pragma unroll
    for (int a = 0; a < 6; ++a) {
        const uint32_t t = wave_reduce_max(m[a]);
        if (l == a) v = t;
        m[a] = 0u;
    }
    if (cur >= 0 && l < 6 && v) atomicMax(&acc[8 * (int64_t)cur + l], v);
}

__global__ __launch_bounds__(DB_THREADS) void db_label_k(const float4* __restrict__ pts,
                                                         const uint32_t* __restrict__ cid,
                                                         const uint8_t* __restrict__ core_s,
                                                         const int* __restrict__ root,
                                                         const int* __restrict__ comp_min,
                                                         const uint32_t* __restrict__ bits,
                                                         const uint32_t* __restrict__ rank, int64_t n,
                                                         const uint32_t* __restrict__ cell_start,
                                                         int* __restrict__ cell_label,
                                                         int32_t* __restrict__ labels,
                                                         uint8_t* __restrict__ core_out, int64_t chunk_size, int bpc,
                                                         int64_t nchunks, uint32_t* __restrict__ box_acc,
                                                         int32_t box_cap) {
    int64_t lo, hi;
    {
        const int64_t woff = (int64_t)wave_id() * (64 * DB_LAB_ROUNDS);
        if (bpc > 0) {
            const int64_t slot = blockIdx.x >> 3;
            const int64_t c = (slot / bpc) * 8 + (blockIdx.x & 7);
            const int64_t within = (slot % bpc) * DB_LAB_TILE + woff;
            lo = c * chunk_size + within;
            hi = (c < nchunks && within < chunk_size) ? (c + 1) * chunk_size : lo;
        } else {
            lo = (int64_t)blockIdx.x * DB_LAB_TILE + woff;
            hi = n;
        }
        if (hi > n) hi = n;
        if (hi > lo + 64 * DB_LAB_ROUNDS) hi = lo + 64 * DB_LAB_ROUNDS;
    }
    if (lo >= hi) return;
    const int l = lane_id();
    constexpr int R = DB_LAB_ROUNDS;
    bool valid[R], is_core[R];
    uint32_t c[R], cs[R], row[R], rk[R], bw[R];
    int rt[R], lab[R];
    float4 p[R];
#pragma unroll
    for (int u = 0; u < R; ++u) {
        const int64_t i = lo + u * 64 + l;
        valid[u] = i < hi;
        c[u] = valid[u] ? cid[i] : 0u;
        p[u] = pts[valid[u] ? i : lo];
        is_core[u] = valid[u] && core_s[i] != 0;
    }
#pragma unroll
    for (int u = 0; u < R; ++u) {
        rt[u] = valid[u] ? root[c[u]] : -1;
        cs[u] = valid[u] ? cell_start[c[u]] : 0xFFFFFFFFu;
    }
#pragma unroll
    for (int u = 0; u < R; ++u) row[u] = rt[u] >= 0 ? (uint32_t)comp_min[rt[u]] : 0u;
#pragma unroll
    for (int u = 0; u < R; ++u) {
        rk[u] = rt[u] >= 0 ? rank[row[u] >> 5] : 0u;
        bw[u] = rt[u] >= 0 ? bits[row[u] >> 5] : 0u;
    }
#pragma unroll
    for (int u = 0; u < R; ++u) {
        const int64_t i = lo + u * 64 + l;
        lab[u] = rt[u] >= 0 ? (int)(rk[u] + (uint32_t)__popc(bw[u] & ((1u << (row[u] & 31u)) - 1u))) : INT_BIG;
        if (valid[u]) {
            const uint32_t o = __float_as_uint(p[u].w);
            labels[o] = is_core[u] ? lab[u] : -1;
            if (core_out) core_out[o] = is_core[u] ? 1 : 0;
            if (cs[u] == (uint32_t)i) cell_label[c[u]] = lab[u];
        }
    }
    if (!box_acc) return;
    int cur = -1;
    uint32_t m[6] = {0u, 0u, 0u, 0u, 0u, 0u};
#pragma unroll
    for (int u = 0; u < R; ++u) {
        const int mine = (is_core[u] && lab[u] != INT_BIG && lab[u] >= 0 && lab[u] < box_cap) ? lab[u] : -1;
        const uint32_t k[3] = {f32_ordered(p[u].x), f32_ordered(p[u].y), f32_ordered(p[u].z)};
        unsigned long long todo = __ballot(mine >= 0);
        while (todo) {
            const int L = __builtin_amdgcn_readlane(mine, (int)__builtin_ctzll(todo));
            const bool in = mine == L;
            todo &= ~__ballot(in);
            if (L != cur) {
                db_box_flush(box_acc, cur, m);
                cur = L;
            }
            if (in) {
#pragma unroll
                for (int a = 0; a < 3; ++a) {
                    m[a] = ~k[a] > m[a] ? ~k[a] : m[a];
                    m[3 + a] = k[a] > m[3 + a] ? k[a] : m[3 + a];
                }
            }
        }
    }
    db_box_flush(box_acc, cur, m);
}

__global__ __launch_bounds__(DB_THREADS) void db_border_k(DbGrid g, const float4* __restrict__ pts,
                                                          const uint32_t* __restrict__ cell_start,
                                                          const uint64_t* __restrict__ cell_key, int m,
                                                          const int2* __restrict__ rowtab,
                                                          const uint8_t* __restrict__ core_s,
                                                          const uint32_t* __restrict__ cell_ncore,
                                                          const float* __restrict__ cell_box,
                                                          const int* __restrict__ cell_label,
                                                          int32_t* __restrict__ labels,
                                                          uint32_t* __restrict__ box_acc, int32_t box_cap) {
    __shared__ RowSet rows[DB_WAVES];
    const int A = blockIdx.x * DB_WAVES + wave_id();
    if (A >= m) return;
    const uint32_t as = cell_start[A], ae = cell_start[A + 1];
    if (cell_ncore[A] == (ae - as)) return;
    const int l = lane_id();
    RowSet* rs = &rows[wave_id()];
    db_rows(g, cell_key, cell_key[A], rs, rowtab, A);
    int any = 0;
    if (l < DB_ROWS)
        for (int B = rs->ca[l]; B < rs->cb[l]; ++B) any |= (cell_ncore[B] != 0);
    if (!__ballot(any != 0)) return;
    constexpr int BR = 3, BROWS = 12;
    int Bc[BR], Bl[BR];
    bool Bd[BR];
    float Bx[BR][6];
#pragma unroll
    for (int rd = 0; rd < BR; ++rd) {
        const int row = rd * BROWS + l / 5, k = l % 5;
        Bc[rd] = -1; Bl[rd] = INT_BIG; Bd[rd] = false;
#pragma unroll
        for (int a = 0; a < 6; ++a) Bx[rd][a] = 0.0f;
        if (l < 5 * BROWS && row < DB_ROWS) {
            const int B = rs->ca[row] + k;
            if (B < rs->cb[row]) {
                const uint32_t nb = cell_ncore[B];
                if (nb != 0) {
                    Bc[rd] = B;
                    Bl[rd] = cell_label[B];
                    Bd[rd] = nb == cell_start[B + 1] - cell_start[B];
#pragma unroll
                    for (int a = 0; a < 6; ++a) Bx[rd][a] = cell_box[6 * (int64_t)B + a];
                }
            }
        }
    }
    for (uint32_t q = as; q < ae; ++q) {
        if (core_s[q]) continue;
        const float4 qp = pts[q];
        bool cand[BR];
#pragma unroll
        for (int rd = 0; rd < BR; ++rd) cand[rd] = Bc[rd] >= 0 && !(db_box_d2(qp, Bx[rd]) > g.eps2);
        int best = INT_BIG;
        for (;;) {
            int mine = INT_BIG, sel = -1;
#pragma unroll
            for (int rd = 0; rd < BR; ++rd)
                if (cand[rd] && Bl[rd] < mine) { mine = Bl[rd]; sel = rd; }
            const int lo = wave_reduce_min(mine);
            if (lo == INT_BIG) break;
            const int owner = (int)__builtin_ctzll(__ballot(mine == lo));
            int Bsel = -1;
            bool dsel = false;
#pragma unroll
            for (int rd = 0; rd < BR; ++rd)
                if (sel == rd) { Bsel = Bc[rd]; dsel = Bd[rd]; }
            const int B = __builtin_amdgcn_readlane(Bsel, owner);
            const bool b_dense = __builtin_amdgcn_readlane((int)dsel, owner) != 0;
            const uint32_t bs = cell_start[B], be = cell_start[B + 1];
            bool found = false;
            for (uint32_t j0 = bs; j0 < be; j0 += 64) {
                const uint32_t j = j0 + l;
                bool hit = false;
                if (j < be && (b_dense || core_s[j])) hit = db_within2(qp, pts[j], g);
                if (__ballot(hit)) { found = true; break; }
            }
            if (found) { best = lo; break; }
            if (l == owner) {
#pragma unroll
                for (int rd = 0; rd < BR; ++rd)
                    if (sel == rd) cand[rd] = false;
            }
        }
        if (l == 0 && best != INT_BIG) labels[__float_as_uint(qp.w)] = best;
        if (box_acc && best != INT_BIG && best >= 0 && best < box_cap && l < 6) {
            const float v = l % 3 == 0 ? qp.x : (l % 3 == 1 ? qp.y : qp.z);
            const uint32_t k = f32_ordered(v);
            atomicMax(&box_acc[8 * (int64_t)best + l], l < 3 ? ~k : k);
        }
    }
}

__global__ __launch_bounds__(DB_THREADS) void db_remap_points_k(const float4* __restrict__ pts,
                                                                const uint8_t* __restrict__ core_s, int64_t n,
                                                                const int32_t* __restrict__ map, int32_t nmap,
                                                                int32_t* __restrict__ labels) {
    const int64_t i = (int64_t)blockIdx.x * DB_THREADS + threadIdx.x;
    if (i >= n) return;
    const uint32_t o = __float_as_uint(pts[i].w);
    int32_t lab = -1;
    if (core_s[i]) {
        const int32_t old = labels[o];
        lab = (old >= 0 && old < nmap) ? map[old] : -1;
    }
    labels[o] = lab;
}
__global__ __launch_bounds__(DB_THREADS) void db_remap_cells_k(int* __restrict__ cell_label,
                                                               const uint32_t* __restrict__ cell_ncore, int m,
                                                               const int32_t* __restrict__ map, int32_t nmap) {
    const int c = blockIdx.x * DB_THREADS + threadIdx.x;
    if (c >= m) return;
    if (cell_ncore[c] == 0) return;
    const int old = cell_label[c];
    const int neu = (old >= 0 && old < nmap) ? map[old] : -1;
    cell_label[c] = neu >= 0 ? neu : INT_BIG;
}

__global__ __launch_bounds__(DB_THREADS) void db_first_rows_k(const uint32_t* __restrict__ bits,
                                                              const uint32_t* __restrict__ rank, int64_t nw,
                                                              int32_t* __restrict__ out) {
    const int64_t i = (int64_t)blockIdx.x * DB_THREADS + threadIdx.x;
    if (i >= nw) return;
    uint32_t b = bits[i];
    uint32_t c = rank[i];
    while (b) {
        const int t = __builtin_ctz(b);
        b &= b - 1;
        out[c++] = (int32_t)(i * 32 + t);
    }
}

__global__ __launch_bounds__(DB_THREADS) void db_strip_pairs_k(const float4* __restrict__ pts,
                                                               const uint32_t* __restrict__ cell_start,
                                                               const uint8_t* __restrict__ core_s,
                                                               const uint32_t* __restrict__ cell_ncore,
                                                               const float* __restrict__ cell_box,
                                                               const int* __restrict__ cell_label, int m, float x_lo,
                                                               float x_hi, int32_t cap, int32_t* __restrict__ out_pairs,
                                                               int32_t* __restrict__ out_count) {
    const int c = blockIdx.x * DB_WAVES + wave_id();
    if (c >= m) return;
    if (cell_ncore[c] == 0) return;
    if (!(cell_box[6 * (int64_t)c + 3] >= x_lo && cell_box[6 * (int64_t)c] < x_hi)) return;
    const int l = lane_id();
    const uint32_t a = cell_start[c], b = cell_start[c + 1];
    uint32_t best = 0xFFFFFFFFu;
    for (uint32_t i = a + l; i < b; i += 64) {
        if (!core_s[i]) continue;
        const float4 p = pts[i];
        if (p.x >= x_lo && p.x < x_hi) {
            const uint32_t row = __float_as_uint(p.w);
            best = row < best ? row : best;
        }
    }
    best = wave_reduce_min(best);
    if (l == 0 && best != 0xFFFFFFFFu) {
        const int32_t slot = atomicAdd(out_count, 1);
        if (slot < cap) {
            out_pairs[2 * slot] = (int32_t)best;
            out_pairs[2 * slot + 1] = cell_label[c];
        }
    }
}

__global__ void db_prelabel_k(const uint32_t* __restrict__ total, int32_t* __restrict__ out_nclusters,
                              uint32_t* __restrict__ box_acc, int64_t box_words) {
    if (threadIdx.x == 0 && blockIdx.x == 0) *out_nclusters = (int32_t)*total;
    const int64_t i = (int64_t)blockIdx.x * blockDim.x + threadIdx.x;
    if (box_acc && i < box_words) box_acc[i] = 0u;
}

struct DbWs {
    uint32_t* meta;
    uint64_t *k0, *k1, *cell_key;
    uint32_t *v0, *v1, *head, *cid, *cell_start, *cell_ncore, *flag, *radix_ws, *scan_ws;
    float4   *pts, *xbuf;
    uint8_t*  core_s;
    float*    cell_box;
    uint32_t* cell_acc;
    int*      cell_min;
    int      *parent, *root, *comp_min, *cell_label;
    int2*     rowtab;
    int64_t   rowtab_cells;
    uint32_t* chunk_bad;
    uint32_t* chunk_ovf;
    uint32_t* chunk_cells;
    uint32_t* comp;
    uint32_t* flag2;
    unsigned long long* core_stats;
    uint32_t* scan1_b;
};

static void db_plan(Arena& a, int64_t n, DbWs& w) {
    const int64_t nn = n > 0 ? n : 1;
    w.meta = a.take<uint32_t>(64);
    w.scan1_b = a.take<uint32_t>(scan1_ws_u32(nn / 32 + 1));
    w.chunk_cells = a.take<uint32_t>(nn + 8);
    w.core_stats = a.take<unsigned long long>(4);
    w.chunk_bad = a.take<uint32_t>(nn + 8);
    w.chunk_ovf = a.take<uint32_t>(nn + 8);
    w.k0 = a.take<uint64_t>(nn);
    w.k1 = a.take<uint64_t>(nn);
    w.v0 = a.take<uint32_t>(nn);
    w.v1 = a.take<uint32_t>(nn);
    w.head = a.take<uint32_t>(nn + 8);
    w.cid = a.take<uint32_t>(nn);
    w.pts = a.take<float4>(nn);
    w.xbuf = a.take<float4>(nn);
    w.core_s = a.take<uint8_t>(nn);
    w.cell_key = a.take<uint64_t>(nn);
    w.cell_start = a.take<uint32_t>(nn + 8);
    w.cell_ncore = a.take<uint32_t>(nn);
    w.cell_box = a.take<float>(6 * nn);
    w.cell_acc = a.take<uint32_t>(8 * nn);
    w.cell_min = a.take<int>(nn);
    w.parent = a.take<int>(nn);
    w.root = a.take<int>(nn);
    w.comp_min = a.take<int>(nn);
    w.cell_label = a.take<int>(nn);
    w.flag = a.take<uint32_t>(nn / 16 + 256);
    w.radix_ws = a.take<uint32_t>(radix_ws_u32(nn));
    w.scan_ws = a.take<uint32_t>(scan_ws_u32(nn));
    w.rowtab_cells = nn / 4 > 65536 ? nn / 4 : (nn < 65536 ? nn : 65536);
    w.rowtab = a.take<int2>((size_t)w.rowtab_cells * DB_ROWS);
    w.comp = a.take<uint32_t>(3 * nn);
    w.flag2 = a.take<uint32_t>(nn + 8);
}

struct DbCells {
    DbGrid g; const float4* pts; const uint32_t* cell_start; const uint64_t* cell_key; int m;
    const int2* rowtab;
    const uint8_t* core_s; const uint32_t* cell_ncore; const float* cell_box;
};
#define DB_GRID_ARGS(c) (c).g, (c).pts, (c).cell_start, (c).cell_key, (c).m, (c).rowtab
#define DB_CELL_ARGS(c) DB_GRID_ARGS(c), (c).core_s, (c).cell_ncore, (c).cell_box

struct DbTuning { int sort_mode; bool no_boxfold, no_xcd, count_pairs; };
static int g_sort_mode = -1;
static thread_local bool g_count_pairs = false;
static DbTuning db_tuning() {
    static const bool no_boxfold = getenv("PCH_DB_NO_BOXFOLD") != nullptr, no_xcd = getenv("PCH_DB_NO_XCD") != nullptr;
    int m = __atomic_load_n(&g_sort_mode, __ATOMIC_RELAXED);
    if (m < 0) {
        const char* e = getenv("PCH_DBSCAN_SORT");
        m = (e && strcmp(e, "chunk") == 0) ? 1 : (e && strcmp(e, "global") == 0) ? 2 : 0;
        __atomic_store_n(&g_sort_mode, m, __ATOMIC_RELAXED);
    }
    return {m, no_boxfold, no_xcd, g_count_pairs};
}

struct DbLastRun { void* ws; size_t ws_bytes; int64_t n; DbCells c; };
static thread_local DbLastRun g_last = {nullptr, 0, 0, {}};

void ws_touched(const void* base, size_t bytes) {
    if (!g_last.ws) return;
    const char* a0 = static_cast<const char*>(base);
    const char* b0 = static_cast<const char*>(g_last.ws);
    if (a0 < b0 + g_last.ws_bytes && b0 < a0 + bytes) g_last.ws = nullptr;
}

static int db_continue(const char* entry, int64_t n, void* ws, size_t ws_bytes, DbWs& w) {
    if (g_last.ws != ws || g_last.ws_bytes != ws_bytes || g_last.n != n || ws == nullptr) {
        set_error("%s must follow pch_dbscan_f32 of this thread on the same, untouched workspace", entry);
        return PCH_ERR_ARG;
    }
    Arena a(ws, ws_bytes, true);
    db_plan(a, n, w);
    return PCH_OK;
}

static float host_unordered(uint32_t k) {
    uint32_t u = (k & 0x80000000u) ? (k & 0x7fffffffu) : ~k;
    float f;
    memcpy(&f, &u, 4);
    return f;
}

static unsigned db_stride_blocks(int64_t n) { return (unsigned)std::min(ceil_div(n, DB_THREADS * 8), int64_t(2048)); }

struct DbRun {
    const float* xyz; int64_t n, chunk_size, nchunks;
    int32_t* labels; uint8_t* core; int32_t* out_nclusters;
    hipStream_t s; DbWs w;
};

static int db_all_noise(const DbRun& r) {
    PCH_HIP_TRY(hipMemsetAsync(r.labels, 0xFF, sizeof(int32_t) * (size_t)r.n, r.s));
    if (r.core) PCH_HIP_TRY(hipMemsetAsync(r.core, 0, (size_t)r.n, r.s));
    PCH_HIP_TRY(hipMemsetAsync(r.out_nclusters, 0, sizeof(int32_t), r.s));
    return PCH_OK;
}

static int db_bounds(const DbRun& r, const float* aabb_host, float (&box)[6], bool& done) {
    if (aabb_host) {
        memcpy(box, aabb_host, sizeof(box));
    } else {
        uint32_t* meta = r.w.meta;
        PCH_HIP_TRY(hipMemsetAsync(meta, 0xFF, 3 * sizeof(uint32_t), r.s));
        PCH_HIP_TRY(hipMemsetAsync(meta + 3, 0, 3 * sizeof(uint32_t), r.s));
        PCH_LAUNCH("db_aabb_in", db_aabb_in_k, dim3(db_stride_blocks(r.n)), dim3(DB_THREADS), 0, r.s, r.xyz, r.n, meta);
        uint32_t mm[6];
        PCH_HIP_TRY(hipMemcpyAsync(mm, meta, sizeof(mm), hipMemcpyDeviceToHost, r.s));
        PCH_HIP_TRY(hipStreamSynchronize(r.s));
        if (mm[0] == 0xFFFFFFFFu) {
            done = true;
            return db_all_noise(r);
        }
        for (int k = 0; k < 6; ++k) box[k] = host_unordered(mm[k]);
    }
    for (int k = 0; k < 6; ++k) {
        if (!(box[k] == box[k]) || box[k] > 3.0e38f || box[k] < -3.0e38f) {
            set_error("bounding box is not finite");
            return PCH_ERR_ARG;
        }
    }
    return PCH_OK;
}

static int db_cell_bits(DbGrid& g, int mx, int my, int mz) {
    g.mx = mx; g.my = my; g.mz = mz;
    g.bx = bits_for((uint64_t)mx + 1); g.by = bits_for((uint64_t)my + 1); g.bz = bits_for((uint64_t)mz + 1);
    return g.bx + g.by + g.bz;
}

static bool db_grid(const DbRun& r, const float (&box)[6], double eps, int32_t min_samples, DbGrid& g, int& cellbits,
                    int& nbits) {
    g.ox = box[0]; g.oy = box[1]; g.oz = box[2];
    g.cell = eps / 1.7320508075688772 * (1.0 - 1.0 / 65536.0);
    g.inv_cell = 1.0 / g.cell;
    g.eps2 = eps * eps;
    g.eps2_lo = nextafterf((float)(g.eps2 * (1.0 - 1.0 / 1048576.0)), -INFINITY);
    g.eps2_hi = nextafterf((float)(g.eps2 * (1.0 + 1.0 / 1048576.0)), INFINITY);
    if (!(g.eps2_hi < 3.0e38f)) { g.eps2_lo = -1.0f; g.eps2_hi = NAN; }
    g.chunk_size = r.chunk_size;
    g.chunk_bad = r.w.chunk_bad;
    g.chunk_cells = r.w.chunk_cells;
    g.min_samples = min_samples;
    int mc[3] = {0, 0, 0};
    bool overflow = false;
    for (int k = 0; k < 3; ++k) {
        const double ext = ((double)box[3 + k] - (double)box[k]) * g.inv_cell;
        if (!(ext < 2.0e9)) overflow = true;
        else mc[k] = (int)ext + 1;
    }
    cellbits = db_cell_bits(g, mc[0], mc[1], mc[2]);
    nbits = cellbits + bits_for((uint64_t)r.nchunks);
    return overflow || nbits > 64;
}

static int db_run_chunks(const DbRun& r, double eps, int32_t min_samples, void* ws, size_t ws_bytes, int32_t* k_host) {
    int32_t offset = 0;
    for (int64_t c = 0; c < r.nchunks; ++c) {
        const int64_t lo = c * r.chunk_size, cn = (r.n - lo) < r.chunk_size ? (r.n - lo) : r.chunk_size;
        int32_t kc = 0;
        PCH_TRY(dbscan_run(r.xyz + 3 * lo, cn, eps, min_samples, 0, nullptr, r.labels + lo,
                           r.core ? r.core + lo : nullptr, r.out_nclusters, ws, ws_bytes, r.s, &kc));
        if (kc > 0 && offset > 0)
            PCH_LAUNCH("db_add_offset", db_add_offset_k, dim3((unsigned)ceil_div(cn, DB_THREADS)), dim3(DB_THREADS), 0,
                       r.s, r.labels + lo, cn, offset);
        offset += kc;
    }
    PCH_HIP_TRY(hipMemcpyAsync(r.out_nclusters, &offset, sizeof(int32_t), hipMemcpyHostToDevice, r.s));
    PCH_HIP_TRY(hipStreamSynchronize(r.s));
    if (k_host) *k_host = offset;
    g_last.ws = nullptr;
    return PCH_OK;
}

static int db_compress(const DbRun& r, DbGrid& g, int& cellbits, bool& done) {
    const DbWs& w = r.w; const hipStream_t s = r.s; const int64_t n = r.n;
    const unsigned gn = (unsigned)ceil_div(n, DB_THREADS);
    int64_t* first_bad = reinterpret_cast<int64_t*>(w.meta + 12);
    PCH_HIP_TRY(hipMemsetAsync(first_bad, 0xFF, sizeof(int64_t), s));
    PCH_LAUNCH("db_first_bad", db_first_bad_k, dim3(db_stride_blocks(n)), dim3(DB_THREADS), 0, s, r.xyz, n,
               reinterpret_cast<unsigned long long*>(first_bad));
    PCH_HIP_TRY(hipMemsetAsync(w.meta + 6, 0, 6 * sizeof(uint32_t), s));
    for (int axis = 0; axis < 3; ++axis) {
        PCH_LAUNCH("dbc_axis_keys", dbc_axis_keys_k, dim3(gn), dim3(DB_THREADS), 0, s, r.xyz, n, axis, w.k0, w.v0);
        PCH_TRY(radix_sort_pairs(w.k0, w.v0, w.k1, w.v1, n, 32, w.radix_ws, s));
        const bool in1 = radix_sort_result_buffer(32) == 1;
        const uint64_t* ksa = in1 ? w.k1 : w.k0;
        const uint32_t* vsa = in1 ? w.v1 : w.v0;
        PCH_LAUNCH("dbc_heads", dbc_heads_k, dim3(gn), dim3(DB_THREADS), 0, s, ksa, n, g.inv_cell, w.flag2);
        PCH_TRY(scan_exclusive_u32(w.flag2, w.head, n, w.scan_ws, nullptr, s));
        PCH_HIP_TRY(hipMemsetAsync(w.cell_start, 0, sizeof(uint32_t) * (size_t)(n + 8), s));
        for (int phase = 0; phase < 2; ++phase)
            PCH_LAUNCH("dbc_local", dbc_local_k, dim3(gn), dim3(DB_THREADS), 0, s, ksa, w.flag2, w.head, n, g.inv_cell,
                       w.cell_box, phase, w.cid, w.cell_start, w.meta + 6);
        PCH_TRY(scan_exclusive_u32(w.cell_start, w.cell_start, n, w.scan_ws, nullptr, s));
        PCH_LAUNCH("dbc_comp", dbc_comp_k, dim3(gn), dim3(DB_THREADS), 0, s, vsa, w.flag2, w.head, w.cid, w.cell_start,
                   n, axis, w.comp, w.meta + 9);
    }
    uint32_t back[8];
    PCH_HIP_TRY(hipMemcpyAsync(back, w.meta + 6, sizeof(back), hipMemcpyDeviceToHost, s));
    PCH_HIP_TRY(hipStreamSynchronize(s));
    int64_t bad_row;
    memcpy(&bad_row, &back[6], sizeof(bad_row));
    if (bad_row >= 0) {
        PCH_TRY(db_all_noise(r));
        g_last.ws = nullptr;
        done = true;
        return PCH_OK;
    }
    if (back[0] != 0) { set_error("compressed cell coordinates out of range"); return PCH_ERR_RANGE; }
    cellbits = db_cell_bits(g, (int)back[3], (int)back[4], (int)back[5]);
    if (cellbits > 64) {
        set_error("cell key needs %d bits even with compressed coordinates (%lld isolated points?)", cellbits, (long long)n);
        return PCH_ERR_RANGE;
    }
    return PCH_OK;
}

static int db_sorted_keys(const DbRun& r, const DbGrid& g, int cellbits, int nbits, bool compressed, int sort_mode,
                          const uint64_t*& ks) {
    const DbWs& w = r.w; const hipStream_t s = r.s; const int64_t n = r.n, nchunks = r.nchunks;
    const unsigned gn = (unsigned)ceil_div(n, DB_THREADS);
    const size_t bytes = (size_t)(reinterpret_cast<char*>(w.chunk_cells + nchunks + 1) - reinterpret_cast<char*>(w.meta + 4));
    PCH_HIP_TRY(hipMemsetAsync(w.meta + 4, 0, (bytes + 15) & ~size_t(15), s));
    if (!compressed && cellbits <= 31 && r.chunk_size <= CS_MAX_CHUNK && sort_mode != 2 &&
        (sort_mode == 1 || nchunks >= CS_MIN_CHUNKS)) {
        PCH_LAUNCH("db_cellscatter", db_cellscatter_k, dim3((unsigned)nchunks), dim3(CS_THREADS), 0, s, r.xyz, n, g,
                   w.chunk_bad, w.chunk_ovf, w.pts, w.k1, w.meta + 6);
        PCH_LAUNCH("db_chunksort", db_chunksort_k, dim3((unsigned)nchunks), dim3(CS_THREADS), 0, s, r.xyz, n, g,
                   w.chunk_ovf, w.chunk_bad, w.xbuf, w.pts, w.k1, w.meta + 6, (unsigned long long*)w.cell_box);
#ifdef PCH_CS_STAMPS
        {
            unsigned long long t[11];
            PCH_HIP_TRY(hipStreamSynchronize(s));
            PCH_HIP_TRY(hipMemcpy(t, w.cell_box, sizeof(t), hipMemcpyDeviceToHost));
            for (int q = 1; q <= 6; ++q)
                fprintf(stderr, "chunksort phase %d: %.2f us\n", q, (double)(long long)(t[q] - t[q - 1]) / 100.0);
            fprintf(stderr, "chunksort tiles: rank %.2f us, offsets %.2f us, scatter %.2f us\n", (double)t[8] / 100.0,
                    (double)t[9] / 100.0, (double)t[10] / 100.0);
        }
#endif
        ks = w.k1;
        return PCH_OK;
    }
    PCH_HIP_TRY(hipMemsetAsync(w.chunk_bad, 0, sizeof(uint32_t) * (size_t)(nchunks + 1), s));
    if (compressed) {
        PCH_LAUNCH("db_keys_comp", db_keys_comp_k, dim3(gn), dim3(DB_THREADS), 0, s, w.comp, n, g, w.k0, w.v0);
    } else {
        PCH_LAUNCH("db_chunkbad", db_chunkbad_k, dim3(db_stride_blocks(n)), dim3(DB_THREADS), 0, s, r.xyz, n,
                   r.chunk_size, w.chunk_bad);
        PCH_LAUNCH("db_keys", db_keys_k, dim3(gn), dim3(DB_THREADS), 0, s, r.xyz, n, g, w.chunk_bad, w.k0, w.v0,
                   w.meta + 6);
    }
    PCH_TRY(radix_sort_pairs(w.k0, w.v0, w.k1, w.v1, n, nbits, w.radix_ws, s));
    const bool in1 = radix_sort_result_buffer(nbits) == 1;
    ks = in1 ? w.k1 : w.k0;
    PCH_LAUNCH("db_gather", db_gather_k, dim3(gn), dim3(DB_THREADS), 0, s, r.xyz, ks, in1 ? w.v1 : w.v0, n, w.pts);
    return PCH_OK;
}

static int db_cells_core(const DbRun& r, const DbGrid& g, int cellbits, const uint64_t* ks, bool count_pairs,
                         DbCells& c) {
    const DbWs& w = r.w; const hipStream_t s = r.s; const int64_t n = r.n;
    const int64_t ntile = ceil_div(n, (int64_t)SCAN_TILE);
    PCH_LAUNCH("db_heads", db_heads_k, dim3((unsigned)ntile), dim3(DB_THREADS), 0, s, ks, n, w.scan_ws);
    PCH_TRY(scan_tile_sums_u32(w.scan_ws, ntile, w.meta + 7, s));
    uint32_t st_m[2];
    PCH_TRY(peek_enqueue(w.meta + 6, sizeof(st_m), s));
    PCH_LAUNCH("db_cells", db_cells_k, dim3((unsigned)ntile), dim3(DB_THREADS), 0, s, ks, w.scan_ws, n, cellbits,
               r.nchunks, w.cid, w.cell_start, w.cell_key, w.chunk_cells, w.cell_acc);
    PCH_TRY(peek_wait(st_m, sizeof(st_m)));
    if (st_m[0] != 0) {
        set_error("finite coordinates outside the supplied bounding box");
        return PCH_ERR_ARG;
    }
    const int m = (int)st_m[1];
    const unsigned gc = (unsigned)ceil_div(m, DB_WAVES);
    c = {g, w.pts, w.cell_start, w.cell_key, m, m <= w.rowtab_cells ? w.rowtab : nullptr, w.core_s, w.cell_ncore,
         w.cell_box};
    if (c.rowtab)
        PCH_LAUNCH("db_rowtab", db_rowtab_k, dim3((unsigned)ceil_div(m, 2 * DB_WAVES)), dim3(DB_THREADS), 0, s, g,
                   w.cell_key, m, w.rowtab);
    if (count_pairs) {
        PCH_HIP_TRY(hipMemsetAsync(w.core_stats, 0, 4 * sizeof(unsigned long long), s));
        PCH_LAUNCH("db_core_counting", db_core_k<true>, dim3(gc), dim3(DB_THREADS), 0, s, DB_GRID_ARGS(c), w.core_s,
                   w.cell_ncore, w.core_stats);
    } else {
        PCH_LAUNCH("db_core", db_core_k<false>, dim3(gc), dim3(DB_THREADS), 0, s, DB_GRID_ARGS(c), w.core_s,
                   w.cell_ncore, nullptr);
    }
    PCH_LAUNCH("db_cellstats", db_cellstats_k, dim3((unsigned)ceil_div(n, (int64_t)DB_WAVES * 64 * DB_CS_ROUNDS)),
               dim3(DB_THREADS), 0, s, w.pts, w.cid, w.core_s, n, w.cell_acc, w.flag, ceil_div(n, 32));
    PCH_LAUNCH("db_cellfin", db_cellfin_k, dim3((unsigned)ceil_div(m, DB_THREADS)), dim3(DB_THREADS), 0, s,
               w.cell_acc, m, w.cell_box, w.cell_min, w.parent, w.comp_min);
    return PCH_OK;
}

static int db_union(const DbRun& r, const DbCells& c) {
    const DbWs& w = r.w; const hipStream_t s = r.s; const int m = c.m;
    const unsigned gc = (unsigned)ceil_div(m, DB_WAVES);
    const uint8_t* face_todo = nullptr;
    if (c.rowtab) {
        PCH_LAUNCH("db_union_pairs", db_union_pairs_k, dim3((unsigned)ceil_div(4 * (int64_t)m, DB_THREADS)),
                   dim3(DB_THREADS), 0, s, DB_CELL_ARGS(c), w.parent, reinterpret_cast<uint8_t*>(w.root));
        face_todo = reinterpret_cast<const uint8_t*>(w.root);
    }
    PCH_LAUNCH("db_union0", db_union_face_k, dim3(gc), dim3(DB_THREADS), 0, s, DB_CELL_ARGS(c), w.parent, face_todo);
    PCH_LAUNCH("db_flatten", db_flatten_k, dim3((unsigned)ceil_div(m, DB_THREADS)), dim3(DB_THREADS), 0, s,
               w.parent, m);
    PCH_LAUNCH("db_union1", db_union_k, dim3(gc), dim3(DB_THREADS), 0, s, DB_CELL_ARGS(c), w.parent);
    PCH_LAUNCH("db_compmin", db_compmin_k, dim3((unsigned)ceil_div(m, DB_THREADS)), dim3(DB_THREADS), 0, s,
               w.cell_min, w.cell_ncore, m, w.parent, w.root, w.comp_min);
    return PCH_OK;
}

static int db_labels(const DbRun& r, const DbCells& c, const DbTuning& tune, int32_t* k_host, DbBoxOut* boxes) {
    const DbWs& w = r.w; const hipStream_t s = r.s; const int64_t n = r.n, nchunks = r.nchunks; const int m = c.m;
    const int64_t nw = ceil_div(n, 32);
    uint32_t* bits = w.flag;
    uint32_t* wrank = w.flag + ((nw + 63) & ~int64_t(63));
    static_assert(DB_CS_ROUNDS * 64 * DB_WAVES / DB_THREADS <= 32, "db_cellstats_k's grid has a thread per bitmap word");
    PCH_LAUNCH("db_mark", db_mark_k, dim3((unsigned)ceil_div(m, DB_THREADS)), dim3(DB_THREADS), 0, s,
               w.root, w.comp_min, m, bits);
    if (scan1_pays(nw)) PCH_TRY(scan1_exclusive_popc_u32(bits, wrank, nw, w.scan1_b, w.meta + 8, s));
    else PCH_TRY(scan_exclusive_popc_u32(bits, wrank, nw, w.scan_ws, w.meta + 8, s));
    uint32_t* box_acc = (boxes && boxes->acc && boxes->cap > 0 && !tune.no_boxfold) ? boxes->acc : nullptr;
    const int32_t box_cap = box_acc ? boxes->cap : 0;
    PCH_LAUNCH("db_prelabel", db_prelabel_k, dim3((unsigned)(box_acc ? ceil_div(8 * (int64_t)box_cap, 256) : 1)),
               dim3(256), 0, s, w.meta + 8, r.out_nclusters, box_acc, 8 * (int64_t)box_cap);
    if (k_host) PCH_TRY(peek_enqueue(r.out_nclusters, sizeof(int32_t), s));
    const int bpc = (nchunks >= 16 && !tune.no_xcd) ? (int)ceil_div(r.chunk_size, DB_LAB_TILE) : 0;
    const unsigned gl = bpc > 0 ? (unsigned)(8 * ceil_div(nchunks, 8) * bpc) : (unsigned)ceil_div(n, DB_LAB_TILE);
    PCH_LAUNCH("db_label", db_label_k, dim3(gl), dim3(DB_THREADS), 0, s, w.pts, w.cid, w.core_s, w.root, w.comp_min,
               bits, wrank, n, w.cell_start, w.cell_label, r.labels, r.core, r.chunk_size, bpc, nchunks, box_acc,
               box_cap);
    PCH_LAUNCH("db_border", db_border_k, dim3((unsigned)ceil_div(m, DB_WAVES)), dim3(DB_THREADS), 0, s,
               DB_CELL_ARGS(c), w.cell_label, r.labels, box_acc, box_cap);
    if (box_acc) boxes->done = true;
    if (k_host) {
        PCH_TRY(peek_wait(k_host, sizeof(int32_t)));
        if (*k_host < 0) {
            set_error("stage C: a device-side look-back wait ran out of its budget; outputs are undefined");
            return PCH_ERR_TIMEOUT;
        }
    }
    return PCH_OK;
}

}

using namespace pch;

extern "C" int pch_first_nonfinite_row_f32(const float* xyz, int64_t n, int64_t* out_row, void* stream) {
    PCH_DEVICE_GUARD(out_row);
    hipStream_t s = (hipStream_t)stream;
    PCH_REQUIRE(n >= 0 && out_row && (n == 0 || xyz), "bad argument");
    PCH_HIP_TRY(hipMemsetAsync(out_row, 0xFF, sizeof(int64_t), s));
    if (n == 0) return PCH_OK;
    PCH_LAUNCH("db_first_bad", db_first_bad_k, dim3(db_stride_blocks(n)), dim3(DB_THREADS), 0, s, xyz, n,
               reinterpret_cast<unsigned long long*>(out_row));
    return PCH_OK;
}

extern "C" void pch_dbscan_set_sort_mode(int mode) {
    __atomic_store_n(&g_sort_mode, (mode == 1 || mode == 2) ? mode : 0, __ATOMIC_RELAXED);
}

extern "C" size_t pch_dbscan_ws_bytes(int64_t n) {
    if (n < 0) return 0;
    Arena a;
    DbWs w;
    db_plan(a, n, w);
    return a.off;
}

int pch::dbscan_run(const float* xyz, int64_t n, double eps, int32_t min_samples, int64_t chunk_size,
                    const float* aabb_host, int32_t* labels, uint8_t* core, int32_t* out_nclusters, void* ws,
                    size_t ws_bytes, hipStream_t s, int32_t* k_host, DbBoxOut* boxes) {
    if (k_host) *k_host = 0;
    if (boxes) boxes->done = false;
    PCH_REQUIRE(n >= 0 && n < (int64_t(1) << 31), "n out of range [0, 2^31)");
    PCH_REQUIRE(eps > 0.0, "eps must be > 0 (sklearn: InvalidParameterError)");
    PCH_REQUIRE(min_samples >= 1, "min_samples must be >= 1 (sklearn: InvalidParameterError)");
    PCH_REQUIRE(out_nclusters != nullptr, "out_nclusters is null");
    if (n == 0) {
        PCH_HIP_TRY(hipMemsetAsync(out_nclusters, 0, sizeof(int32_t), s));
        return PCH_OK;
    }
    PCH_REQUIRE(xyz && labels && ws, "null buffer");
    Arena a(ws, ws_bytes);
    DbWs w;
    db_plan(a, n, w);
    if (a.overflow) { set_error("workspace too small: need %zu bytes", a.off); return PCH_ERR_WORKSPACE; }
    if (chunk_size <= 0 || chunk_size > n) chunk_size = n;
    const DbRun r = {xyz, n, chunk_size, ceil_div(n, chunk_size), labels, core, out_nclusters, s, w};
    const DbTuning tune = db_tuning();

    float box[6];
    bool done = false;
    PCH_TRY(db_bounds(r, aabb_host, box, done));
    if (done) return PCH_OK;
    DbGrid g;
    int cellbits, nbits;
    const bool overflow = db_grid(r, box, eps, min_samples, g, cellbits, nbits);
    if (overflow) {
        if (r.nchunks > 1) return db_run_chunks(r, eps, min_samples, ws, ws_bytes, k_host);
        PCH_TRY(db_compress(r, g, cellbits, done));
        if (done) return PCH_OK;
        nbits = cellbits;
    }
    const uint64_t* ks;
    DbCells c;
    PCH_TRY(db_sorted_keys(r, g, cellbits, nbits, overflow, tune.sort_mode, ks));
    PCH_TRY(db_cells_core(r, g, cellbits, ks, tune.count_pairs, c));
    PCH_TRY(db_union(r, c));
    PCH_TRY(db_labels(r, c, tune, k_host, boxes));
    g_last = {ws, ws_bytes, n, c};
    return PCH_OK;
}

extern "C" int pch_dbscan_first_core_rows_i32(int64_t n, int32_t* out_rows, void* ws, size_t ws_bytes, void* stream) {
    PCH_DEVICE_GUARD(out_rows ? (const void*)out_rows : (const void*)ws);
    PCH_REQUIRE(n >= 0, "bad argument");
    if (n == 0) return PCH_OK;
    DbWs w;
    PCH_TRY(db_continue(__func__, n, ws, ws_bytes, w));
    PCH_REQUIRE(out_rows != nullptr, "null output");
    const int64_t nw = ceil_div(n, 32);
    const uint32_t* bits = w.flag;
    const uint32_t* wrank = w.flag + ((nw + 63) & ~int64_t(63));
    PCH_LAUNCH("db_first_rows", db_first_rows_k, dim3((unsigned)ceil_div(nw, DB_THREADS)), dim3(DB_THREADS), 0,
               (hipStream_t)stream, bits, wrank, nw, out_rows);
    return PCH_OK;
}

extern "C" void pch_dbscan_set_pair_counting(int enable) { g_count_pairs = enable != 0; }

extern "C" int pch_dbscan_pair_stats(int64_t n, uint64_t* out4_host, void* ws, size_t ws_bytes, void* stream) {
    PCH_DEVICE_GUARD(ws);
    PCH_REQUIRE(n >= 0 && out4_host, "bad argument");
    memset(out4_host, 0, 4 * sizeof(uint64_t));
    if (n == 0) return PCH_OK;
    DbWs w;
    PCH_TRY(db_continue(__func__, n, ws, ws_bytes, w));
    PCH_HIP_TRY(hipMemcpyAsync(out4_host, w.core_stats, 4 * sizeof(uint64_t), hipMemcpyDeviceToHost, (hipStream_t)stream));
    PCH_HIP_TRY(hipStreamSynchronize((hipStream_t)stream));
    return PCH_OK;
}

extern "C" int pch_dbscan_strip_pairs_i32(int64_t n, float x_lo, float x_hi, int32_t cap, int32_t* out_pairs,
                                          int32_t* out_count, void* ws, size_t ws_bytes, void* stream) {
    PCH_DEVICE_GUARD(out_count);
    hipStream_t s = (hipStream_t)stream;
    PCH_REQUIRE(n >= 0 && cap >= 0 && out_count && (cap == 0 || out_pairs), "bad argument");
    PCH_HIP_TRY(hipMemsetAsync(out_count, 0, sizeof(int32_t), s));
    if (n == 0 || !(x_lo < x_hi)) return PCH_OK;
    DbWs w;
    PCH_TRY(db_continue(__func__, n, ws, ws_bytes, w));
    const int m = g_last.c.m;
    PCH_LAUNCH("db_strip_pairs", db_strip_pairs_k, dim3((unsigned)ceil_div(m, DB_WAVES)), dim3(DB_THREADS), 0, s,
               w.pts, w.cell_start, w.core_s, w.cell_ncore, w.cell_box, w.cell_label, m, x_lo, x_hi, cap, out_pairs,
               out_count);
    return PCH_OK;
}

extern "C" int pch_dbscan_relabel_i32(const int32_t* map, int32_t nmap, int64_t n, int32_t* labels, void* ws,
                                      size_t ws_bytes, void* stream) {
    PCH_DEVICE_GUARD(labels);
    hipStream_t s = (hipStream_t)stream;
    PCH_REQUIRE(n >= 0 && nmap >= 0 && (nmap == 0 || map) && (n == 0 || labels), "bad argument");
    if (n == 0) return PCH_OK;
    DbWs w;
    PCH_TRY(db_continue(__func__, n, ws, ws_bytes, w));
    const DbCells& c = g_last.c;
    PCH_LAUNCH("db_remap_points", db_remap_points_k, dim3((unsigned)ceil_div(n, DB_THREADS)), dim3(DB_THREADS), 0, s,
               w.pts, w.core_s, n, map, nmap, labels);
    PCH_LAUNCH("db_remap_cells", db_remap_cells_k, dim3((unsigned)ceil_div(c.m, DB_THREADS)), dim3(DB_THREADS), 0, s,
               w.cell_label, w.cell_ncore, c.m, map, nmap);
    PCH_LAUNCH("db_border", db_border_k, dim3((unsigned)ceil_div(c.m, DB_WAVES)), dim3(DB_THREADS), 0, s,
               DB_CELL_ARGS(c), w.cell_label, labels, nullptr, 0);
    return PCH_OK;
}

extern "C" int pch_dbscan_f32(const float* xyz, int64_t n, double eps, int32_t min_samples,
                              int64_t chunk_size, const float* aabb_host, int32_t* labels,
                              uint8_t* core, int32_t* out_nclusters, void* ws, size_t ws_bytes,
                              void* stream) {
    PCH_DEVICE_GUARD(xyz ? (const void*)xyz : (const void*)out_nclusters);
    return dbscan_run(xyz, n, eps, min_samples, chunk_size, aabb_host, labels, core, out_nclusters, ws, ws_bytes,
                      (hipStream_t)stream, nullptr);
}
```

pointcloudhookup_amd/csrc/pch_lookback.h:

```cpp
#pragma once
#include "pch_common.h"

namespace pch {

constexpr int GF_LOOK = 4;
constexpr uint64_t GF_FLAG_AGG = 1ull << 62, GF_FLAG_INCL = 2ull << 62, GF_FLAG_POISON = 3ull << 62;
constexpr unsigned long long GF_LB_BUDGET = 400000000ull;
constexpr uint32_t GF_LB_FAILED = 0xFFFFFFFFu;

__device__ __forceinline__ void gf_announce(uint64_t* __restrict__ status, int64_t b, uint32_t T) {
    __hip_atomic_store(&status[b], (b == 0 ? GF_FLAG_INCL : GF_FLAG_AGG) | T, __ATOMIC_RELAXED, __HIP_MEMORY_SCOPE_AGENT);
}
__device__ __forceinline__ uint32_t gf_lookback(uint64_t* __restrict__ status, int64_t b, uint32_t T,
                                                bool announced = false, unsigned long long budget = GF_LB_BUDGET) {
    const int l = lane_id();
    if (b == 0) {
        if (l == 0 && !announced) __hip_atomic_store(&status[0], GF_FLAG_INCL | T, __ATOMIC_RELAXED, __HIP_MEMORY_SCOPE_AGENT);
        return 0;
    }
    if (l == 0 && !announced) __hip_atomic_store(&status[b], GF_FLAG_AGG | T, __ATOMIC_RELAXED, __HIP_MEMORY_SCOPE_AGENT);
    uint32_t excl = 0;
    bool done = false;
    unsigned long long t_first_miss = 0;
#ifdef PCH_LB_COUNT
    extern __device__ unsigned long long g_lb_polls, g_lb_windows;
#endif
    for (int64_t j = b - 1; !done; j -= 64 * GF_LOOK) {
#ifdef PCH_LB_COUNT
        if (l == 0) atomicAdd(&g_lb_windows, 1ull);
#endif
        uint64_t v[GF_LOOK];
        bool failed = false;
        do {
            bool missing = false, poisoned = false;
#pragma unroll
            for (int k = 0; k < GF_LOOK; ++k) {
                const int64_t idx = j - 64 * k - l;
                v[k] = idx >= 0 ? __hip_atomic_load(&status[idx], __ATOMIC_RELAXED, __HIP_MEMORY_SCOPE_AGENT)
                                : GF_FLAG_INCL;
                missing |= (v[k] >> 62) == 0;
                poisoned |= (v[k] >> 62) == 3;
            }
            if (__ballot(poisoned) != 0) { failed = true; break; }
            if (__ballot(missing) == 0) break;
#ifdef PCH_LB_COUNT
            if (l == 0) atomicAdd(&g_lb_polls, 1ull);
#endif
            const unsigned long long now = wall_clock64();
            if (t_first_miss == 0) t_first_miss = now | 1ull;
            else if (now - t_first_miss > budget) { failed = true; break; }
            __builtin_amdgcn_s_sleep(1);
        } while (true);
        if (failed) {
            if (l == 0) __hip_atomic_store(&status[b], GF_FLAG_POISON, __ATOMIC_RELAXED, __HIP_MEMORY_SCOPE_AGENT);
            return GF_LB_FAILED;
        }
#pragma unroll
        for (int k = 0; k < GF_LOOK; ++k) {
            if (done) break;
            const unsigned long long incl = __ballot((v[k] >> 62) == 2);
            if (incl) {
                const int first = (int)__builtin_ctzll(incl);
                excl += wave_reduce_add(l <= first ? (uint32_t)v[k] : 0u);
                done = true;
            } else {
                excl += wave_reduce_add((uint32_t)v[k]);
            }
        }
    }
    if (l == 0) __hip_atomic_store(&status[b], GF_FLAG_INCL | (uint64_t)(excl + T), __ATOMIC_RELAXED,
                                   __HIP_MEMORY_SCOPE_AGENT);
    return excl;
}


}
```

pointcloudhookup_amd/csrc/pch_pipeline.hip:

```cpp
#include "pch_common.h"

#include <cstring>

namespace pch {

struct DevInfo {
    float   scalars[8];
    float   aabb[6];
    float   pad[2];
    int64_t count;
    int32_t nclusters;
    int32_t pad2;
};

static size_t max3(size_t a, size_t b, size_t c) { return a > b ? (a > c ? a : c) : (b > c ? b : c); }

}

using namespace pch;

extern "C" size_t pch_tower_clusters_ws_bytes(int64_t n, int64_t nf_cap, int32_t k_cap) {
    if (n < 0 || nf_cap < 0 || k_cap < 0) return 0;
    Arena a;
    a.take<DevInfo>(1);
    return a.off + max3(pch_ground_filter_ws_bytes(n), pch_dbscan_ws_bytes(nf_cap),
                        pch_segment_by_label_ws_bytes(nf_cap, k_cap));
}

extern "C" int pch_tower_clusters_f32(const float* raw, int64_t n, double pct, float offset,
                                      float fallback_offset, int64_t min_keep, double eps,
                                      int32_t min_samples, int64_t chunk_size, float* out_points,
                                      int32_t* out_index, int32_t* out_labels, int32_t* out_perm,
                                      int64_t* out_offsets, float* out_stats, int64_t nf_cap,
                                      int32_t k_cap, PchTowerClusters* info_host, void* ws,
                                      size_t ws_bytes, void* stream) {
    hipStream_t s = (hipStream_t)stream;
    PCH_DEVICE_GUARD(raw);
    PCH_REQUIRE(info_host != nullptr, "info_host is null");
    memset(info_host, 0, sizeof(*info_host));
    PCH_REQUIRE(ws != nullptr && nf_cap >= 0 && k_cap >= 0, "bad argument");
    Arena a(ws, ws_bytes);
    DevInfo* dev = a.take<DevInfo>(1);
    if (a.overflow || ws_bytes < pch_tower_clusters_ws_bytes(n, nf_cap, k_cap)) {
        set_error("workspace too small: need %zu bytes", pch_tower_clusters_ws_bytes(n, nf_cap, k_cap));
        return PCH_ERR_WORKSPACE;
    }
    void* sub = static_cast<char*>(ws) + a.off;
    const size_t sub_bytes = ws_bytes - a.off;

    static_assert(sizeof(DevInfo) <= 256, "fits the pinned peek buffer");
    const GfEarly early = {dev, sizeof(DevInfo)};
    PCH_TRY(ground_filter_run(raw, n, pct, offset, fallback_offset, min_keep, out_points, out_index,
                              dev->scalars, &dev->count, dev->aabb, sub, sub_bytes, s, &early));
    DevInfo h;
    PCH_TRY(peek_wait(&h, sizeof(DevInfo)));
    if (h.scalars[5] != 0.0f && h.count >= 0) {
        PCH_TRY(peek_enqueue(dev, sizeof(DevInfo), s));
        PCH_TRY(peek_wait(&h, sizeof(DevInfo)));
    }
    memcpy(info_host->centroid, h.scalars, 3 * sizeof(float));
    info_host->base = h.scalars[3];
    info_host->threshold = h.scalars[4];
    info_host->used_fallback = h.scalars[5] != 0.0f;
    {
        uint32_t c0;
        memcpy(&c0, &h.scalars[6], sizeof(c0));
        info_host->count_at_offset = (int64_t)c0;
    }
    memcpy(info_host->aabb, h.aabb, sizeof(h.aabb));
    info_host->count = h.count;
    const int64_t nf = h.count;
    if (nf < 0) {
        set_error("stage B: a device-side look-back wait ran out of its budget; outputs are undefined");
        return PCH_ERR_TIMEOUT;
    }
    if (nf > nf_cap) {
        set_error("the filter kept %lld points, more than nf_cap = %lld", (long long)nf, (long long)nf_cap);
        return PCH_ERR_WORKSPACE;
    }
    if (nf == 0) {
        if (out_offsets) PCH_HIP_TRY(hipMemsetAsync(out_offsets, 0, sizeof(int64_t), s));
        return PCH_OK;
    }
    PCH_REQUIRE(out_labels != nullptr, "out_labels is null");
    int32_t k = 0;
    DbBoxOut box = {reinterpret_cast<uint32_t*>(out_stats), (out_perm && out_offsets && out_stats) ? k_cap : 0, false};
    PCH_TRY(dbscan_run(out_points, nf, eps, min_samples, chunk_size, h.aabb, out_labels, nullptr,
                       &dev->nclusters, sub, sub_bytes, s, &k, &box));
    info_host->nclusters = k;
    if (out_perm && out_offsets) {
        if (k > k_cap) {
            set_error("%d clusters found, more than k_cap = %d (labels are valid; group them with "
                      "pch_segment_by_label)", (int)k, (int)k_cap);
            return PCH_ERR_RANGE;
        }
        PCH_TRY(segment_run(out_labels, out_points, nf, k, out_perm, out_offsets, out_stats, sub, sub_bytes, s,
                            box.done));
    }
    return PCH_OK;
}
```

pointcloudhookup_amd/csrc/pch_segment.hip:

```cpp
#include "pch_prims.h"

namespace pch {

constexpr int SG_THREADS = 256;

__global__ __launch_bounds__(SG_THREADS) void sg_keys_k(const int32_t* __restrict__ labels, int64_t n,
                                                        int32_t nclusters, uint64_t* __restrict__ keys,
                                                        uint32_t* __restrict__ vals) {
    const int64_t i = (int64_t)blockIdx.x * SG_THREADS + threadIdx.x;
    if (i >= n) return;
    const int32_t l = labels[i];
    keys[i] = (l < 0 || l >= nclusters) ? (uint64_t)nclusters : (uint64_t)l;
    vals[i] = (uint32_t)i;
}

__device__ __forceinline__ void sg_decode_word(uint32_t* enc, int64_t i) {
    const int a = (int)(i & 7);
    const uint32_t u = enc[i];
    uint32_t v = 0u;
    if (a < 3) v = u == 0u ? 0x7F800000u : __float_as_uint(f32_unordered(~u));
    else if (a < 6) v = u == 0u ? 0xFF800000u : __float_as_uint(f32_unordered(u));
    enc[i] = v;
}

__global__ __launch_bounds__(SG_THREADS) void sg_offsets_k(const uint64_t* __restrict__ keys, int64_t n,
                                                           int32_t nclusters, int64_t* __restrict__ offsets,
                                                           uint32_t* enc_stats) {
    const int64_t k = (int64_t)blockIdx.x * SG_THREADS + threadIdx.x;
    if (enc_stats && k < 8 * (int64_t)nclusters) sg_decode_word(enc_stats, k);
    if (k > nclusters) return;
    int64_t lo = 0, hi = n;
    while (lo < hi) { const int64_t mid = (lo + hi) >> 1; if (keys[mid] < (uint64_t)k) lo = mid + 1; else hi = mid; }
    offsets[k] = lo;
}

__global__ __launch_bounds__(SG_THREADS) void sg_perm_k(const uint32_t* __restrict__ vals, int64_t n,
                                                        int32_t* __restrict__ perm) {
    const int64_t i = (int64_t)blockIdx.x * SG_THREADS + threadIdx.x;
    if (i < n) perm[i] = (int32_t)vals[i];
}

__global__ __launch_bounds__(SG_THREADS) void sg_stats_init_k(uint32_t* __restrict__ acc, int32_t nclusters) {
    const int i = blockIdx.x * SG_THREADS + threadIdx.x;
    if (i < 6 * nclusters) acc[i] = (i % 6) < 3 ? 0xFFFFFFFFu : 0u;
}

__device__ __forceinline__ void sg_flush(uint32_t* __restrict__ acc, int cur, const uint32_t (&lo)[3],
                                         const uint32_t (&hi)[3]) {
    const int l = lane_id();
    if (cur >= 0 && l < 6) {
        uint32_t v = 0;
#pragma unroll
        for (int a = 0; a < 3; ++a) { if (l == a) v = lo[a]; if (l == 3 + a) v = hi[a]; }
        if (l < 3) atomicMin(&acc[6 * (int64_t)cur + l], v);
        else       atomicMax(&acc[6 * (int64_t)cur + l], v);
    }
}

__global__ __launch_bounds__(SG_THREADS) void sg_stats_k(const float* __restrict__ xyz,
                                                         const int32_t* __restrict__ labels, int64_t n,
                                                         int32_t nclusters, uint32_t* __restrict__ acc) {
    const int64_t w = (int64_t)blockIdx.x * (SG_THREADS / 64) + wave_id();
    const int l = lane_id();
    int cur = -1;
    uint32_t lo[3] = {0xFFFFFFFFu, 0xFFFFFFFFu, 0xFFFFFFFFu}, hi[3] = {0u, 0u, 0u};
    struct Row3 { float x, y, z; };
    int lab16[16];
#pragma unroll
    for (int r = 0; r < 16; ++r) {
        const int64_t j = w * 1024 + r * 64 + l;
        const int v = j < n ? labels[j] : -1;
        lab16[r] = (v >= 0 && v < nclusters) ? v : -1;
    }
    for (int r = 0; r < 16; ++r) {
        const int64_t j = w * 1024 + r * 64 + l;
        const int lab = lab16[r];
        uint32_t k[3] = {0, 0, 0};
        if (lab >= 0) {
            const Row3 q = reinterpret_cast<const Row3*>(xyz)[j];
            k[0] = f32_ordered(q.x); k[1] = f32_ordered(q.y); k[2] = f32_ordered(q.z);
        }
        unsigned long long todo = __ballot(lab >= 0);
        while (todo) {
            const int lead = (int)__builtin_ctzll(todo);
            const int L = __builtin_amdgcn_readlane(lab, lead);
            const unsigned long long same = __ballot(lab == L);
            todo &= ~same;
            if (L != cur) {
                sg_flush(acc, cur, lo, hi);
#pragma unroll
                for (int a = 0; a < 3; ++a) { lo[a] = 0xFFFFFFFFu; hi[a] = 0u; }
                cur = L;
            }
#pragma unroll
            for (int a = 0; a < 3; ++a) {
                const uint32_t mn = wave_reduce_min(lab == L ? k[a] : 0xFFFFFFFFu);
                const uint32_t mx = wave_reduce_max(lab == L ? k[a] : 0u);
                lo[a] = mn < lo[a] ? mn : lo[a];
                hi[a] = mx > hi[a] ? mx : hi[a];
            }
        }
    }
    sg_flush(acc, cur, lo, hi);
}

constexpr int SL_ROUNDS = 8;
constexpr int SL_TILE   = SG_THREADS * SL_ROUNDS;

__device__ __forceinline__ uint32_t sl_bin(int32_t l, int32_t nclusters) {
    return (l < 0 || l >= nclusters) ? (uint32_t)nclusters : (uint32_t)l;
}

__global__ __launch_bounds__(SG_THREADS) void sl_hist_k(const int32_t* __restrict__ labels, int64_t n,
                                                        int32_t nclusters, uint32_t* __restrict__ hist,
                                                        int64_t nb, uint32_t* __restrict__ zero_ws,
                                                        int64_t zero_words) {
    __shared__ uint32_t h[256];
    {
        const int64_t g = (int64_t)blockIdx.x * SG_THREADS + threadIdx.x;
        if (g < zero_words) zero_ws[g] = 0u;
    }
    h[threadIdx.x] = 0;
    __syncthreads();
    const int64_t base = (int64_t)blockIdx.x * SL_TILE;
    int32_t v[SL_ROUNDS];
#pragma unroll
    for (int r = 0; r < SL_ROUNDS; ++r) {
        const int64_t i = base + r * SG_THREADS + threadIdx.x;
        v[r] = i < n ? labels[i] : -1;
    }
#pragma unroll
    for (int r = 0; r < SL_ROUNDS; ++r) {
        const int64_t i = base + r * SG_THREADS + threadIdx.x;
        const bool in = i < n;
        const uint32_t b = sl_bin(v[r], nclusters);
        const unsigned long long act = __ballot(in);
        if (act) {
            const uint32_t b0 = (uint32_t)__builtin_amdgcn_readlane((int)b, (int)__builtin_ctzll(act));
            const unsigned long long same = __ballot(in && b == b0);
            if (lane_id() == (int)__builtin_ctzll(act)) atomicAdd(&h[b0], (uint32_t)__popcll(same));
            if (in && b != b0) atomicAdd(&h[b], 1u);
        }
    }
    __syncthreads();
    if ((int)threadIdx.x <= nclusters) hist[(int64_t)threadIdx.x * nb + blockIdx.x] = h[threadIdx.x];
}

__global__ __launch_bounds__(SG_THREADS) void sl_scatter_k(const int32_t* __restrict__ labels, int64_t n,
                                                           int32_t nclusters,
                                                           const uint32_t* __restrict__ offs, int64_t nb,
                                                           int32_t* __restrict__ perm) {
    constexpr int WAVES = SG_THREADS / 64;
    __shared__ uint32_t cnt[WAVES][256];
    const int w = wave_id(), l = lane_id();
    for (int j = threadIdx.x; j < WAVES * 256; j += SG_THREADS) (&cnt[0][0])[j] = 0;
    __syncthreads();
    const int64_t seg = (int64_t)blockIdx.x * SL_TILE + (int64_t)w * (64 * SL_ROUNDS);
    uint32_t bin[SL_ROUNDS], rank[SL_ROUNDS];
    const uint64_t lt = lanemask_lt();
#pragma unroll
    for (int r = 0; r < SL_ROUNDS; ++r) {
        const int64_t i = seg + r * 64 + l;
        bin[r] = sl_bin(i < n ? labels[i] : -1, nclusters);
    }
#pragma unroll
    for (int r = 0; r < SL_ROUNDS; ++r) {
        const bool valid = seg + r * 64 + l < n;
        const uint32_t d = bin[r];
        uint64_t peers = __ballot(valid);
#pragma unroll
        for (int b = 0; b < 8; ++b) {
            const bool bit = (d >> b) & 1u;
            const uint64_t m = __ballot(bit);
            peers &= bit ? m : ~m;
        }
        const uint32_t prior = cnt[w][d];
        const uint32_t rk = (uint32_t)__popcll(peers & lt);
        __builtin_amdgcn_wave_barrier();
        if (valid && rk == 0) cnt[w][d] = prior + (uint32_t)__popcll(peers);
        __builtin_amdgcn_wave_barrier();
        rank[r] = prior + rk;
    }
    __syncthreads();
    if ((int)threadIdx.x <= nclusters) {
        const int d = threadIdx.x;
        uint32_t run = offs[(int64_t)d * nb + blockIdx.x];
#pragma unroll
        for (int w2 = 0; w2 < WAVES; ++w2) {
            const uint32_t c = cnt[w2][d];
            cnt[w2][d] = run;
            run += c;
        }
    }
    __syncthreads();
#pragma unroll
    for (int r = 0; r < SL_ROUNDS; ++r) {
        const int64_t i = seg + r * 64 + l;
        if (i < n) perm[cnt[w][bin[r]] + rank[r]] = (int32_t)i;
    }
}

__global__ __launch_bounds__(SG_THREADS) void sl_offsets_k(const uint32_t* __restrict__ offs, int64_t nb,
                                                           int32_t nclusters, int64_t* __restrict__ offsets,
                                                           uint32_t* enc_stats, const uint32_t* __restrict__ scan_total) {
    const int k = blockIdx.x * SG_THREADS + threadIdx.x;
    const bool failed = scan_total && *scan_total == 0xFFFFFFFFu;
    if (k <= nclusters) offsets[k] = failed ? int64_t(-1) : (int64_t)offs[(int64_t)k * nb];
    if (enc_stats && k < 8 * nclusters) sg_decode_word(enc_stats, k);
}

__global__ __launch_bounds__(SG_THREADS) void sg_stats_out_k(const uint32_t* __restrict__ acc, int32_t nclusters,
                                                             float* __restrict__ stats) {
    const int i = blockIdx.x * SG_THREADS + threadIdx.x;
    if (i >= 8 * nclusters) return;
    const int k = i >> 3, a = i & 7;
    float v = 0.0f;
    if (a < 6) {
        const uint32_t u = acc[6 * (int64_t)k + a];
        const bool empty = a < 3 ? (u == 0xFFFFFFFFu) : (u == 0u);
        v = empty ? (a < 3 ? INFINITY : -INFINITY) : f32_unordered(u);
    }
    stats[i] = v;
}

struct SgWs {
    uint64_t *k0, *k1;
    uint32_t *v0, *v1, *radix_ws, *acc;
    uint32_t *table, *table_scan;
};
static void sg_plan(Arena& a, int64_t n, int32_t nclusters, SgWs& w) {
    const int64_t nn = n > 0 ? n : 1;
    w.acc = a.take<uint32_t>(6 * (size_t)(nclusters > 0 ? nclusters : 1));
    if (nclusters < 256) {
        const int64_t table = ((int64_t)nclusters + 1) * ceil_div(nn, SL_TILE);
        w.table = a.take<uint32_t>(table);
        w.table_scan = a.take<uint32_t>(scan1_pays(table) ? scan1_ws_u32(table) : scan_ws_u32(table));
        w.k0 = w.k1 = nullptr; w.v0 = w.v1 = w.radix_ws = nullptr;
    } else {
        w.table = w.table_scan = nullptr;
        w.k0 = a.take<uint64_t>(nn);
        w.k1 = a.take<uint64_t>(nn);
        w.v0 = a.take<uint32_t>(nn);
        w.v1 = a.take<uint32_t>(nn);
        w.radix_ws = a.take<uint32_t>(radix_ws_u32(nn));
    }
}

}

using namespace pch;

extern "C" size_t pch_segment_by_label_ws_bytes(int64_t n, int32_t nclusters) {
    if (n < 0) return 0;
    Arena a;
    SgWs w;
    sg_plan(a, n, nclusters, w);
    return a.off;
}

extern "C" int pch_segment_by_label(const int32_t* labels, const float* xyz, int64_t n,
                                    int32_t nclusters, int32_t* out_perm, int64_t* out_offsets,
                                    float* out_stats, void* ws, size_t ws_bytes, void* stream) {
    PCH_DEVICE_GUARD(labels ? (const void*)labels : (const void*)out_offsets);
    return segment_run(labels, xyz, n, nclusters, out_perm, out_offsets, out_stats, ws, ws_bytes, (hipStream_t)stream,
                       false);
}

int pch::segment_run(const int32_t* labels, const float* xyz, int64_t n, int32_t nclusters, int32_t* out_perm,
                     int64_t* out_offsets, float* out_stats, void* ws, size_t ws_bytes, hipStream_t s,
                     bool stats_encoded) {
    PCH_REQUIRE(n >= 0 && n < (int64_t(1) << 31) && nclusters >= 0, "bad size");
    PCH_REQUIRE(out_offsets != nullptr, "out_offsets is null");
    if (n == 0) {
        PCH_HIP_TRY(hipMemsetAsync(out_offsets, 0, sizeof(int64_t) * ((size_t)nclusters + 1), s));
        return PCH_OK;
    }
    PCH_REQUIRE(labels && out_perm && ws, "null buffer");
    PCH_REQUIRE(!out_stats || xyz, "stats requested without coordinates");
    Arena a(ws, ws_bytes);
    SgWs w;
    sg_plan(a, n, nclusters, w);
    if (a.overflow) { set_error("workspace too small: need %zu bytes", a.off); return PCH_ERR_WORKSPACE; }
    const unsigned gn = (unsigned)ceil_div(n, SG_THREADS);
    if (nclusters < 256) {
        const int64_t nb = ceil_div(n, SL_TILE);
        const int64_t table = ((int64_t)nclusters + 1) * nb;
        const bool one = scan1_pays(table);
        const int64_t zero_words = one ? (int64_t)scan1_ws_u32(table) : 0;
        PCH_REQUIRE(zero_words <= nb * SG_THREADS, "count table too large for the fused zeroing");
        PCH_LAUNCH("seg_hist", sl_hist_k, dim3((unsigned)nb), dim3(SG_THREADS), 0, s, labels, n, nclusters,
                   w.table, nb, w.table_scan, zero_words);
        const uint32_t* scan_total = one ? w.table_scan + 2 * ceil_div(table, (int64_t)SCAN_TILE) + 1 : nullptr;
        if (one) PCH_TRY(scan1_exclusive_u32(w.table, w.table, table, w.table_scan, const_cast<uint32_t*>(scan_total), s));
        else PCH_TRY(scan_exclusive_u32(w.table, w.table, table, w.table_scan, nullptr, s));
        PCH_LAUNCH("seg_scatter", sl_scatter_k, dim3((unsigned)nb), dim3(SG_THREADS), 0, s, labels, n, nclusters,
                   (const uint32_t*)w.table, nb, out_perm);
        PCH_LAUNCH("seg_offsets", sl_offsets_k,
                   dim3((unsigned)ceil_div(stats_encoded ? 8 * (int64_t)nclusters + 1 : (int64_t)nclusters + 1, SG_THREADS)),
                   dim3(SG_THREADS), 0, s, (const uint32_t*)w.table, nb, nclusters, out_offsets,
                   stats_encoded ? reinterpret_cast<uint32_t*>(out_stats) : (uint32_t*)nullptr, scan_total);
    } else {
        PCH_LAUNCH("seg_keys", sg_keys_k, dim3(gn), dim3(SG_THREADS), 0, s, labels, n, nclusters, w.k0, w.v0);
        const int nbits = bits_for((uint64_t)nclusters + 1);
        PCH_TRY(radix_sort_pairs(w.k0, w.v0, w.k1, w.v1, n, nbits, w.radix_ws, s));
        const bool in1 = radix_sort_result_buffer(nbits) == 1;
        const uint64_t* ks = in1 ? w.k1 : w.k0;
        const uint32_t* vs = in1 ? w.v1 : w.v0;
        PCH_LAUNCH("seg_perm", sg_perm_k, dim3(gn), dim3(SG_THREADS), 0, s, vs, n, out_perm);
        PCH_LAUNCH("seg_offsets", sg_offsets_k,
                   dim3((unsigned)ceil_div(stats_encoded ? 8 * (int64_t)nclusters + 1 : (int64_t)nclusters + 1, SG_THREADS)),
                   dim3(SG_THREADS), 0, s, ks, n, nclusters, out_offsets,
                   stats_encoded ? reinterpret_cast<uint32_t*>(out_stats) : (uint32_t*)nullptr);
    }
    if (out_stats && nclusters > 0 && !stats_encoded) {
        PCH_LAUNCH("seg_stats_init", sg_stats_init_k, dim3((unsigned)ceil_div(6 * (int64_t)nclusters, SG_THREADS)),
                   dim3(SG_THREADS), 0, s, w.acc, nclusters);
        PCH_LAUNCH("seg_stats", sg_stats_k, dim3((unsigned)ceil_div(n, 1024 * (SG_THREADS / 64))), dim3(SG_THREADS),
                   0, s, xyz, labels, n, nclusters, w.acc);
        PCH_LAUNCH("seg_stats_out", sg_stats_out_k, dim3((unsigned)ceil_div(8 * (int64_t)nclusters, SG_THREADS)),
                   dim3(SG_THREADS), 0, s, (const uint32_t*)w.acc, nclusters, out_stats);
    }
    return PCH_OK;
}
```

profiles/summarize.py:

```python
#!/usr/bin/env python3
import collections
import csv
import glob
import json
import os
import sys

tag, stats_dir, fetch_dir, write_dir, points = sys.argv[1:6]
kind = sys.argv[6] if len(sys.argv) > 6 else "corridor"
frame = sys.argv[7] if len(sys.argv) > 7 else "offset"
sq_dirs = sys.argv[8:]
here = os.path.dirname(os.path.abspath(__file__))


def short(name):
    name = name.replace("void ", "")
    return name.split("(")[0].replace("pch::", "")


rows = list(csv.DictReader(open(glob.glob(os.path.join(stats_dir, "**/*kernel_stats.csv"), recursive=True)[0])))
ours = [r for r in rows if "pch::" in r["Name"]]
with open(os.path.join(here, f"{tag}_kernel_stats.csv"), "w") as f:
    f.write("kernel,calls,avg_us,min_us,max_us,total_ms,percent_of_all_gpu_time\n")
    for r in sorted(ours, key=lambda r: -float(r["TotalDurationNs"])):
        f.write(f"{short(r['Name'])},{r['Calls']},{float(r['AverageNs']) / 1e3:.2f},{float(r['MinNs']) / 1e3:.2f},"
                f"{float(r['MaxNs']) / 1e3:.2f},{float(r['TotalDurationNs']) / 1e6:.3f},{r['Percentage']}\n")


def pmc(d, counter):
    acc = collections.defaultdict(list)
    for r in csv.DictReader(open(glob.glob(os.path.join(d, "**/*counter_collection.csv"), recursive=True)[0])):
        if r["Counter_Name"] == counter and "pch::" in r["Kernel_Name"]:
            acc[short(r["Kernel_Name"])].append(float(r["Counter_Value"]))
    return acc


fetch, write = pmc(fetch_dir, "FETCH_SIZE"), pmc(write_dir, "WRITE_SIZE")
steps_in_stats = 6
steps_in_pmc = 3
names = {"ms_summary_k": "mean_summary", "ms_walk_k": "mean_walk", "ms_level2_k": "mean_level2",
         "db_core_k": "db_core", "db_core_k<false>": "db_core", "db_core_k<true>": "db_core_counting",
         "db_union_pairs_k": "db_union_pairs", "db_mark_k": "db_mark", "sel_bracket_k": "sel_bracket",
         "sg_hist_k": "seg_hist", "sg_scatter_k": "seg_scatter", "db_union_k": "db_union", "db_border_k": "db_border",
         "gf_compact_k<0>": "gf_compact", "gf_compact_k<1>": "gf_compact_fb", "db_chunksort_k": "db_chunksort", "db_cellscatter_k": "db_cellscatter",
         "sel_hist_k<0, 1, true>": "sel_hist0",
         "sel_hist_k<1, 1, true>": "sel_hist1", "sel_hist_k<2, 1, true>": "sel_hist2", "rs_scatter_k": "radix_scatter",
         "rs_hist_k": "radix_hist", "db_gather_k": "db_gather", "db_keys_k": "db_keys",
         "sg_stats_k": "seg_stats", "db_label_k": "db_label", "db_cellbox_k": "db_cellbox",
         "db_union_face_k": "db_union0", "db_rowtab_k": "db_rowtab", "db_cellstats_k": "db_cellstats",
         "db_cells_k": "db_cells", "ms_sample_k": "mean_sample", "ms_prefix_k": "mean_prefix",
         "scan1_k<false>": "scan1", "scan1_k<true>": "scan1_popc", "db_prelabel_k": "db_prelabel",
         "sl_hist_k": "seg_hist", "sl_scatter_k": "seg_scatter", "sl_offsets_k": "seg_offsets",
         "vx_finish_k": "voxel_finish", "vx_scatter_k": "voxel_scatter", "vx_scatter_lds_k": "voxel_scatter",
         "vx_tilehist_k": "voxel_tilehist", "vx_minmax_k": "voxel_minmax", "vx_split_k": "voxel_split",
         "vx_binscan_k": "voxel_binscan"}
sys.path.insert(0, here)
from stamp import csrc_sha
traffic = {"points": int(points), "kind": kind, "frame": frame, "source": tag, "csrc_sha": csrc_sha(),
           "unit": "bytes per launch (2*FETCH_SIZE + WRITE_SIZE, KiB->B)", "kernels": {}}
with open(os.path.join(here, f"{tag}_pmc_traffic.csv"), "w") as f:
    f.write("kernel,launches,fetch_bytes_raw_per_launch,fetch_bytes_x2_per_launch,write_bytes_per_launch\n")
    for k in sorted(set(fetch) | set(write), key=lambda k: -sum(fetch.get(k, [0]))):
        fl, wl = fetch.get(k, []), write.get(k, [])
        fb = 1024 * sum(fl) / max(len(fl), 1)
        wb = 1024 * sum(wl) / max(len(wl), 1)
        f.write(f"{k},{max(len(fl), len(wl))},{fb:.0f},{2 * fb:.0f},{wb:.0f}\n")
        if k in names:
            traffic["kernels"][names[k]] = int(2 * fb + wb)
traffic["launches_per_step"] = round(sum(int(r["Calls"]) for r in ours) / steps_in_stats, 2)
traffic["kernel_ms_per_step"] = round(sum(float(r["TotalDurationNs"]) for r in ours) / 1e6 / steps_in_stats, 4)
tot = 0.0
for k in set(fetch) | set(write):
    tot += 1024 * (2 * sum(fetch.get(k, [])) + sum(write.get(k, [])))
traffic["step_bytes"] = int(tot / steps_in_pmc)
traffic["avg_us"] = {names.get(short(r["Name"]), short(r["Name"])): round(float(r["AverageNs"]) / 1e3, 2) for r in ours}
if sq_dirs:
    sq = collections.defaultdict(dict)
    for d in sq_dirs:
        files = glob.glob(os.path.join(d, "**/*counter_collection.csv"), recursive=True)
        if not files:
            continue
        acc = collections.defaultdict(lambda: collections.defaultdict(list))
        for r in csv.DictReader(open(files[0])):
            if "pch::" in r["Kernel_Name"]:
                acc[short(r["Kernel_Name"])][r["Counter_Name"]].append(float(r["Counter_Value"]))
        for k, cs in acc.items():
            for c, v in cs.items():
                sq[k][c] = sum(v) / max(len(v), 1)
    cols = sorted({c for v in sq.values() for c in v})
    with open(os.path.join(here, f"{tag}_sq_counters.csv"), "w") as f:
        f.write("kernel," + ",".join(cols) + ",avg_us,valu_issue_frac\n")
        dur = {short(r["Name"]): float(r["AverageNs"]) / 1e3 for r in ours}
        for k in sorted(sq, key=lambda k: -sq[k].get("SQ_INSTS_VALU", 0)):
            us = dur.get(k, 0.0)
            frac = sq[k].get("SQ_INSTS_VALU", 0) * 4 / (1024 * 2.4e9 * us * 1e-6) if us else 0.0
            f.write(k + "," + ",".join(f"{sq[k].get(c, 0):.0f}" for c in cols) + f",{us:.2f},{frac:.4f}\n")
            if k in names:
                traffic.setdefault("sq", {})[names[k]] = dict({c: int(sq[k].get(c, 0)) for c in cols},
                                                               valu_issue_frac=round(frac, 4))
tpath = os.path.join(here, "traffic.json")
try:
    allt = json.load(open(tpath))
    if "workloads" not in allt:
        allt = {"workloads": {}}
except Exception:
    allt = {"workloads": {}}
allt["workloads"][f"{kind}/{frame}/{int(points)}"] = traffic
json.dump(allt, open(tpath, "w"), indent=1)
print(open(os.path.join(here, f"{tag}_pmc_traffic.csv")).read())
```

Measured before the change: 61180.

## Replace segment hist/scan/scatter with decoupled look-back sweep and DBSCAN-fused cluster counts

Replaces the small-cluster segment path (per-tile histogram, global scan of the count table, scatter, offsets kernels) with at most 256 large tiles. Each tile counts its labels and then runs a decoupled look-back over per-bin tile aggregates to scatter the permutation in one sweep kernel. The DBSCAN labeling and border kernels now also accumulate per-cluster sizes into the box accumulator, and the prelabel kernel zeroes the sweep control area. When that has happened the count pass is skipped and only the sweep runs. This removes several launches and the large count-table scan, at the cost of spin-waiting look-back with a timeout and poison fallback, plus extra atomics inside the DBSCAN kernels.

```diff
diff --git a/pointcloudhookup_amd/csrc/pch_common.h b/pointcloudhookup_amd/csrc/pch_common.h
--- a/pointcloudhookup_amd/csrc/pch_common.h
+++ b/pointcloudhookup_amd/csrc/pch_common.h
@@ -81,7 +81,9 @@
 int peek_enqueue(const void* dev, size_t bytes, hipStream_t s);
 int peek_wait(void* dst, size_t bytes);
 
-struct DbBoxOut { uint32_t* acc; int32_t cap; bool done; };
+struct DbBoxOut { uint32_t* acc; int32_t cap; bool done; uint32_t* zero; int64_t zero_words; bool zeroed; };
+constexpr int    SEG_MAX_TILES = 256, SEG_CTL_WORDS = 64;
+constexpr size_t SEG_SWEEP_WORDS = SEG_CTL_WORDS + 256 * (size_t)SEG_MAX_TILES;
 struct GfEarly { const void* dev; size_t bytes; };
 int ground_filter_run(const float* raw, int64_t n, double pct, float offset, float fallback_offset, int64_t min_keep,
                       float* out_points, int32_t* out_index, float* out_scalars, int64_t* out_count, float* out_aabb,
@@ -90,7 +92,8 @@
                const float* aabb_host, int32_t* labels, uint8_t* core, int32_t* out_nclusters,
                void* ws, size_t ws_bytes, hipStream_t s, int32_t* k_host, DbBoxOut* box = nullptr);
 int segment_run(const int32_t* labels, const float* xyz, int64_t n, int32_t nclusters, int32_t* out_perm,
-                int64_t* out_offsets, float* out_stats, void* ws, size_t ws_bytes, hipStream_t s, bool stats_encoded);
+                int64_t* out_offsets, float* out_stats, void* ws, size_t ws_bytes, hipStream_t s, bool stats_encoded,
+                uint32_t* counted_sweep = nullptr);
 
 bool prof_enabled();
 bool prof_wanted(const char* name);
diff --git a/pointcloudhookup_amd/csrc/pch_dbscan.hip b/pointcloudhookup_amd/csrc/pch_dbscan.hip
--- a/pointcloudhookup_amd/csrc/pch_dbscan.hip
+++ b/pointcloudhookup_amd/csrc/pch_dbscan.hip
@@ -1496,7 +1496,7 @@
 constexpr int DB_LAB_ROUNDS = 8;
 constexpr int DB_LAB_TILE   = DB_THREADS * DB_LAB_ROUNDS;
 
-__device__ __forceinline__ void db_box_flush(uint32_t* __restrict__ acc, int cur, uint32_t (&m)[6]) {
+__device__ __forceinline__ void db_box_flush(uint32_t* __restrict__ acc, int cur, uint32_t (&m)[6], uint32_t& cn) {
     const int l = lane_id();
     uint32_t v = 0;
 #pragma unroll
@@ -1505,7 +1505,10 @@
         if (l == a) v = t;
         m[a] = 0u;
     }
+    const uint32_t c = cn;
+    cn = 0u;
     if (cur >= 0 && l < 6 && v) atomicMax(&acc[8 * (int64_t)cur + l], v);
+    if (cur >= 0 && l == 6 && c) atomicAdd(&acc[8 * (int64_t)cur + 6], c);
 }
 
 __global__ __launch_bounds__(DB_THREADS) void db_label_k(const float4* __restrict__ pts,
@@ -1578,6 +1581,7 @@
     if (!box_acc) return;
     int cur = -1;
     uint32_t m[6] = {0u, 0u, 0u, 0u, 0u, 0u};
+    uint32_t cn = 0u;
 #pragma unroll
     for (int u = 0; u < R; ++u) {
         const int mine = (is_core[u] && lab[u] != INT_BIG && lab[u] >= 0 && lab[u] < box_cap) ? lab[u] : -1;
@@ -1586,11 +1590,13 @@
         while (todo) {
             const int L = __builtin_amdgcn_readlane(mine, (int)__builtin_ctzll(todo));
             const bool in = mine == L;
-            todo &= ~__ballot(in);
+            const unsigned long long inb = __ballot(in);
+            todo &= ~inb;
             if (L != cur) {
-                db_box_flush(box_acc, cur, m);
+                db_box_flush(box_acc, cur, m, cn);
                 cur = L;
             }
+            cn += (uint32_t)__popcll(inb);
             if (in) {
 #pragma unroll
                 for (int a = 0; a < 3; ++a) {
@@ -1600,7 +1606,7 @@
             }
         }
     }
-    db_box_flush(box_acc, cur, m);
+    db_box_flush(box_acc, cur, m, cn);
 }
 
 __global__ __launch_bounds__(DB_THREADS) void db_border_k(DbGrid g, const float4* __restrict__ pts,
@@ -1687,10 +1693,11 @@
             }
         }
         if (l == 0 && best != INT_BIG) labels[__float_as_uint(qp.w)] = best;
-        if (box_acc && best != INT_BIG && best >= 0 && best < box_cap && l < 6) {
+        if (box_acc && best != INT_BIG && best >= 0 && best < box_cap && l < 7) {
             const float v = l % 3 == 0 ? qp.x : (l % 3 == 1 ? qp.y : qp.z);
             const uint32_t k = f32_ordered(v);
-            atomicMax(&box_acc[8 * (int64_t)best + l], l < 3 ? ~k : k);
+            if (l < 6) atomicMax(&box_acc[8 * (int64_t)best + l], l < 3 ? ~k : k);
+            else       atomicAdd(&box_acc[8 * (int64_t)best + 6], 1u);
         }
     }
 }
@@ -1768,10 +1775,12 @@
 }
 
 __global__ void db_prelabel_k(const uint32_t* __restrict__ total, int32_t* __restrict__ out_nclusters,
-                              uint32_t* __restrict__ box_acc, int64_t box_words) {
+                              uint32_t* __restrict__ box_acc, int64_t box_words, uint32_t* __restrict__ zero,
+                              int64_t zero_words) {
     if (threadIdx.x == 0 && blockIdx.x == 0) *out_nclusters = (int32_t)*total;
     const int64_t i = (int64_t)blockIdx.x * blockDim.x + threadIdx.x;
     if (box_acc && i < box_words) box_acc[i] = 0u;
+    if (zero && i < zero_words) zero[i] = 0u;
 }
 
 struct DbWs {
@@ -2124,8 +2133,11 @@
     else PCH_TRY(scan_exclusive_popc_u32(bits, wrank, nw, w.scan_ws, w.meta + 8, s));
     uint32_t* box_acc = (boxes && boxes->acc && boxes->cap > 0 && !tune.no_boxfold) ? boxes->acc : nullptr;
     const int32_t box_cap = box_acc ? boxes->cap : 0;
-    PCH_LAUNCH("db_prelabel", db_prelabel_k, dim3((unsigned)(box_acc ? ceil_div(8 * (int64_t)box_cap, 256) : 1)),
-               dim3(256), 0, s, w.meta + 8, r.out_nclusters, box_acc, 8 * (int64_t)box_cap);
+    uint32_t* zero = box_acc ? boxes->zero : nullptr;
+    const int64_t zero_words = zero ? boxes->zero_words : 0;
+    const int64_t pre_words = 8 * (int64_t)box_cap > zero_words ? 8 * (int64_t)box_cap : zero_words;
+    PCH_LAUNCH("db_prelabel", db_prelabel_k, dim3((unsigned)(pre_words ? ceil_div(pre_words, 256) : 1)),
+               dim3(256), 0, s, w.meta + 8, r.out_nclusters, box_acc, 8 * (int64_t)box_cap, zero, zero_words);
     if (k_host) PCH_TRY(peek_enqueue(r.out_nclusters, sizeof(int32_t), s));
     const int bpc = (nchunks >= 16 && !tune.no_xcd) ? (int)ceil_div(r.chunk_size, DB_LAB_TILE) : 0;
     const unsigned gl = bpc > 0 ? (unsigned)(8 * ceil_div(nchunks, 8) * bpc) : (unsigned)ceil_div(n, DB_LAB_TILE);
@@ -2134,7 +2146,7 @@
                box_cap);
     PCH_LAUNCH("db_border", db_border_k, dim3((unsigned)ceil_div(m, DB_WAVES)), dim3(DB_THREADS), 0, s,
                DB_CELL_ARGS(c), w.cell_label, r.labels, box_acc, box_cap);
-    if (box_acc) boxes->done = true;
+    if (box_acc) { boxes->done = true; boxes->zeroed = zero != nullptr; }
     if (k_host) {
         PCH_TRY(peek_wait(k_host, sizeof(int32_t)));
         if (*k_host < 0) {
@@ -2176,7 +2188,7 @@
                     const float* aabb_host, int32_t* labels, uint8_t* core, int32_t* out_nclusters, void* ws,
                     size_t ws_bytes, hipStream_t s, int32_t* k_host, DbBoxOut* boxes) {
     if (k_host) *k_host = 0;
-    if (boxes) boxes->done = false;
+    if (boxes) boxes->done = boxes->zeroed = false;
     PCH_REQUIRE(n >= 0 && n < (int64_t(1) << 31), "n out of range [0, 2^31)");
     PCH_REQUIRE(eps > 0.0, "eps must be > 0 (sklearn: InvalidParameterError)");
     PCH_REQUIRE(min_samples >= 1, "min_samples must be >= 1 (sklearn: InvalidParameterError)");
diff --git a/pointcloudhookup_amd/csrc/pch_lookback.h b/pointcloudhookup_amd/csrc/pch_lookback.h
--- a/pointcloudhookup_amd/csrc/pch_lookback.h
+++ b/pointcloudhookup_amd/csrc/pch_lookback.h
@@ -73,5 +73,64 @@
     return excl;
 }
 
+constexpr uint32_t GFB_FLAG_AGG = 1u << 30, GFB_FLAG_POISON = 3u << 30, GFB_VALUE = (1u << 30) - 1u;
+__device__ __forceinline__ void gfb_publish(uint32_t* __restrict__ status, int64_t tiles, int d, int64_t b,
+                                            uint32_t count) {
+    __hip_atomic_store(&status[d * tiles + b], GFB_FLAG_AGG | count, __ATOMIC_RELAXED, __HIP_MEMORY_SCOPE_AGENT);
+}
+template <int NB>
+__device__ __forceinline__ bool gfb_sums(uint32_t* __restrict__ status, int64_t tiles, int d0, int dstep, int nbins,
+                                         int64_t b, int64_t upto, uint32_t (&excl)[NB], uint32_t (&total)[NB],
+                                         unsigned long long budget = GF_LB_BUDGET) {
+    const int l = lane_id();
+#pragma unroll
+    for (int q = 0; q < NB; ++q) excl[q] = total[q] = 0u;
+    unsigned long long t_first_miss = 0;
+    bool failed = false;
+    for (int64_t j = 0; j < upto && !failed; j += 64 * GF_LOOK) {
+        uint32_t v[NB][GF_LOOK];
+        do {
+            bool missing = false, poisoned = false;
+#pragma unroll
+            for (int q = 0; q < NB; ++q) {
+                const int d = d0 + q * dstep;
+#pragma unroll
+                for (int k = 0; k < GF_LOOK; ++k) {
+                    const int64_t idx = j + 64 * k + l;
+                    v[q][k] = (d < nbins && idx < upto)
+                                  ? __hip_atomic_load(&status[d * tiles + idx], __ATOMIC_RELAXED, __HIP_MEMORY_SCOPE_AGENT)
+                                  : GFB_FLAG_AGG;
+                    missing |= (v[q][k] >> 30) == 0;
+                    poisoned |= (v[q][k] >> 30) == 3;
+                }
+            }
+            if (__ballot(poisoned) != 0) { failed = true; break; }
+            if (__ballot(missing) == 0) break;
+            const unsigned long long now = wall_clock64();
+            if (t_first_miss == 0) t_first_miss = now | 1ull;
+            else if (now - t_first_miss > budget) { failed = true; break; }
+            __builtin_amdgcn_s_sleep(1);
+        } while (true);
+        if (failed) break;
+#pragma unroll
+        for (int q = 0; q < NB; ++q)
+#pragma unroll
+            for (int k = 0; k < GF_LOOK; ++k) {
+                const uint32_t c = v[q][k] & GFB_VALUE;
+                total[q] += c;
+                excl[q] += (j + 64 * k + l < b) ? c : 0u;
+            }
+    }
+    if (failed) {
+        if (l < NB && d0 + l * dstep < nbins)
+            __hip_atomic_store(&status[(d0 + l * dstep) * tiles + b], GFB_FLAG_POISON, __ATOMIC_RELAXED,
+                               __HIP_MEMORY_SCOPE_AGENT);
+        return false;
+    }
+#pragma unroll
+    for (int q = 0; q < NB; ++q) { excl[q] = wave_reduce_add(excl[q]); total[q] = wave_reduce_add(total[q]); }
+    return true;
+}
+
 
 }
diff --git a/pointcloudhookup_amd/csrc/pch_pipeline.hip b/pointcloudhookup_amd/csrc/pch_pipeline.hip
--- a/pointcloudhookup_amd/csrc/pch_pipeline.hip
+++ b/pointcloudhookup_amd/csrc/pch_pipeline.hip
@@ -23,6 +23,7 @@
     if (n < 0 || nf_cap < 0 || k_cap < 0) return 0;
     Arena a;
     a.take<DevInfo>(1);
+    a.take<uint32_t>(SEG_SWEEP_WORDS);
     return a.off + max3(pch_ground_filter_ws_bytes(n), pch_dbscan_ws_bytes(nf_cap),
                         pch_segment_by_label_ws_bytes(nf_cap, k_cap));
 }
@@ -41,6 +42,7 @@
     PCH_REQUIRE(ws != nullptr && nf_cap >= 0 && k_cap >= 0, "bad argument");
     Arena a(ws, ws_bytes);
     DevInfo* dev = a.take<DevInfo>(1);
+    uint32_t* sweep = a.take<uint32_t>(SEG_SWEEP_WORDS);
     if (a.overflow || ws_bytes < pch_tower_clusters_ws_bytes(n, nf_cap, k_cap)) {
         set_error("workspace too small: need %zu bytes", pch_tower_clusters_ws_bytes(n, nf_cap, k_cap));
         return PCH_ERR_WORKSPACE;
@@ -84,7 +86,8 @@
     }
     PCH_REQUIRE(out_labels != nullptr, "out_labels is null");
     int32_t k = 0;
-    DbBoxOut box = {reinterpret_cast<uint32_t*>(out_stats), (out_perm && out_offsets && out_stats) ? k_cap : 0, false};
+    DbBoxOut box = {reinterpret_cast<uint32_t*>(out_stats), (out_perm && out_offsets && out_stats) ? k_cap : 0, false,
+                    sweep, (int64_t)SEG_SWEEP_WORDS, false};
     PCH_TRY(dbscan_run(out_points, nf, eps, min_samples, chunk_size, h.aabb, out_labels, nullptr,
                        &dev->nclusters, sub, sub_bytes, s, &k, &box));
     info_host->nclusters = k;
@@ -95,7 +98,7 @@
             return PCH_ERR_RANGE;
         }
         PCH_TRY(segment_run(out_labels, out_points, nf, k, out_perm, out_offsets, out_stats, sub, sub_bytes, s,
-                            box.done));
+                            box.done, box.done && box.zeroed ? sweep : nullptr));
     }
     return PCH_OK;
 }
diff --git a/pointcloudhookup_amd/csrc/pch_segment.hip b/pointcloudhookup_amd/csrc/pch_segment.hip
--- a/pointcloudhookup_amd/csrc/pch_segment.hip
+++ b/pointcloudhookup_amd/csrc/pch_segment.hip
@@ -1,4 +1,5 @@
 #include "pch_prims.h"
+#include "pch_lookback.h"
 
 namespace pch {
 
@@ -104,109 +105,188 @@
     sg_flush(acc, cur, lo, hi);
 }
 
-constexpr int SL_ROUNDS = 8;
-constexpr int SL_TILE   = SG_THREADS * SL_ROUNDS;
+constexpr int SW_THREADS = 1024, SW_WAVES = SW_THREADS / 64, SW_ROUNDS = 8;
+constexpr int SW_SUB  = SW_THREADS * SW_ROUNDS;
+constexpr int SW_UNIT = 1024;
+constexpr int SW_NB   = 4;
+static_assert(SW_WAVES * SW_NB * 4 >= 256, "four look-back rounds cover every bin");
+
+struct SwPlan { int64_t span, tiles; };
+static SwPlan sw_plan(int64_t n) {
+    SwPlan p;
+    p.span = ceil_div(ceil_div(n, SEG_MAX_TILES), SW_UNIT) * SW_UNIT;
+    p.tiles = ceil_div(n, p.span);
+    return p;
+}
 
 __device__ __forceinline__ uint32_t sl_bin(int32_t l, int32_t nclusters) {
     return (l < 0 || l >= nclusters) ? (uint32_t)nclusters : (uint32_t)l;
 }
 
-__global__ __launch_bounds__(SG_THREADS) void sl_hist_k(const int32_t* __restrict__ labels, int64_t n,
-                                                        int32_t nclusters, uint32_t* __restrict__ hist,
-                                                        int64_t nb, uint32_t* __restrict__ zero_ws,
-                                                        int64_t zero_words) {
+__device__ __forceinline__ void sl_hist(const int32_t* __restrict__ labels, int64_t lo, int64_t hi, int32_t nclusters,
+                                        uint32_t* h) {
+    int32_t v[SW_ROUNDS], nx[SW_ROUNDS];
+#pragma unroll
+    for (int r = 0; r < SW_ROUNDS; ++r) {
+        const int64_t i = lo + r * SW_THREADS + threadIdx.x;
+        nx[r] = i < hi ? labels[i] : -1;
+    }
+    for (int64_t base = lo; base < hi; base += SW_SUB) {
+#pragma unroll
+        for (int r = 0; r < SW_ROUNDS; ++r) {
+            v[r] = nx[r];
+            const int64_t i = base + SW_SUB + r * SW_THREADS + threadIdx.x;
+            nx[r] = i < hi ? labels[i] : -1;
+        }
+#pragma unroll
+        for (int r = 0; r < SW_ROUNDS; ++r) {
+            const int64_t i = base + r * SW_THREADS + threadIdx.x;
+            const bool in = i < hi;
+            const uint32_t b = sl_bin(v[r], nclusters);
+            const unsigned long long act = __ballot(in);
+            if (act) {
+                const uint32_t b0 = (uint32_t)__builtin_amdgcn_readlane((int)b, (int)__builtin_ctzll(act));
+                const unsigned long long same = __ballot(in && b == b0);
+                if (lane_id() == (int)__builtin_ctzll(act)) atomicAdd(&h[b0], (uint32_t)__popcll(same));
+                if (in && b != b0) atomicAdd(&h[b], 1u);
+            }
+        }
+    }
+}
+
+__global__ __launch_bounds__(SW_THREADS) void sl_count_k(const int32_t* __restrict__ labels, int64_t n,
+                                                         int32_t nclusters, int64_t span, int64_t tiles,
+                                                         uint32_t* __restrict__ ctl) {
     __shared__ uint32_t h[256];
-    {
-        const int64_t g = (int64_t)blockIdx.x * SG_THREADS + threadIdx.x;
-        if (g < zero_words) zero_ws[g] = 0u;
-    }
-    h[threadIdx.x] = 0;
-    __syncthreads();
-    const int64_t base = (int64_t)blockIdx.x * SL_TILE;
-    int32_t v[SL_ROUNDS];
-#pragma unroll
-    for (int r = 0; r < SL_ROUNDS; ++r) {
-        const int64_t i = base + r * SG_THREADS + threadIdx.x;
-        v[r] = i < n ? labels[i] : -1;
-    }
-#pragma unroll
-    for (int r = 0; r < SL_ROUNDS; ++r) {
-        const int64_t i = base + r * SG_THREADS + threadIdx.x;
-        const bool in = i < n;
-        const uint32_t b = sl_bin(v[r], nclusters);
-        const unsigned long long act = __ballot(in);
-        if (act) {
-            const uint32_t b0 = (uint32_t)__builtin_amdgcn_readlane((int)b, (int)__builtin_ctzll(act));
-            const unsigned long long same = __ballot(in && b == b0);
-            if (lane_id() == (int)__builtin_ctzll(act)) atomicAdd(&h[b0], (uint32_t)__popcll(same));
-            if (in && b != b0) atomicAdd(&h[b], 1u);
-        }
-    }
-    __syncthreads();
-    if ((int)threadIdx.x <= nclusters) hist[(int64_t)threadIdx.x * nb + blockIdx.x] = h[threadIdx.x];
-}
-
-__global__ __launch_bounds__(SG_THREADS) void sl_scatter_k(const int32_t* __restrict__ labels, int64_t n,
-                                                           int32_t nclusters,
-                                                           const uint32_t* __restrict__ offs, int64_t nb,
-                                                           int32_t* __restrict__ perm) {
-    constexpr int WAVES = SG_THREADS / 64;
-    __shared__ uint32_t cnt[WAVES][256];
-    const int w = wave_id(), l = lane_id();
-    for (int j = threadIdx.x; j < WAVES * 256; j += SG_THREADS) (&cnt[0][0])[j] = 0;
-    __syncthreads();
-    const int64_t seg = (int64_t)blockIdx.x * SL_TILE + (int64_t)w * (64 * SL_ROUNDS);
-    uint32_t bin[SL_ROUNDS], rank[SL_ROUNDS];
-    const uint64_t lt = lanemask_lt();
-#pragma unroll
-    for (int r = 0; r < SL_ROUNDS; ++r) {
-        const int64_t i = seg + r * 64 + l;
-        bin[r] = sl_bin(i < n ? labels[i] : -1, nclusters);
-    }
-#pragma unroll
-    for (int r = 0; r < SL_ROUNDS; ++r) {
-        const bool valid = seg + r * 64 + l < n;
-        const uint32_t d = bin[r];
-        uint64_t peers = __ballot(valid);
-#pragma unroll
-        for (int b = 0; b < 8; ++b) {
-            const bool bit = (d >> b) & 1u;
-            const uint64_t m = __ballot(bit);
-            peers &= bit ? m : ~m;
-        }
-        const uint32_t prior = cnt[w][d];
-        const uint32_t rk = (uint32_t)__popcll(peers & lt);
-        __builtin_amdgcn_wave_barrier();
-        if (valid && rk == 0) cnt[w][d] = prior + (uint32_t)__popcll(peers);
-        __builtin_amdgcn_wave_barrier();
-        rank[r] = prior + rk;
-    }
-    __syncthreads();
-    if ((int)threadIdx.x <= nclusters) {
-        const int d = threadIdx.x;
-        uint32_t run = offs[(int64_t)d * nb + blockIdx.x];
-#pragma unroll
-        for (int w2 = 0; w2 < WAVES; ++w2) {
-            const uint32_t c = cnt[w2][d];
-            cnt[w2][d] = run;
-            run += c;
-        }
-    }
-    __syncthreads();
-#pragma unroll
-    for (int r = 0; r < SL_ROUNDS; ++r) {
-        const int64_t i = seg + r * 64 + l;
-        if (i < n) perm[cnt[w][bin[r]] + rank[r]] = (int32_t)i;
-    }
-}
-
-__global__ __launch_bounds__(SG_THREADS) void sl_offsets_k(const uint32_t* __restrict__ offs, int64_t nb,
-                                                           int32_t nclusters, int64_t* __restrict__ offsets,
-                                                           uint32_t* enc_stats, const uint32_t* __restrict__ scan_total) {
-    const int k = blockIdx.x * SG_THREADS + threadIdx.x;
-    const bool failed = scan_total && *scan_total == 0xFFFFFFFFu;
-    if (k <= nclusters) offsets[k] = failed ? int64_t(-1) : (int64_t)offs[(int64_t)k * nb];
-    if (enc_stats && k < 8 * nclusters) sg_decode_word(enc_stats, k);
+    if (blockIdx.x == 0 && threadIdx.x < SEG_CTL_WORDS) ctl[threadIdx.x] = 0u;
+    if (threadIdx.x < 256) h[threadIdx.x] = 0;
+    __syncthreads();
+    const int64_t b = blockIdx.x, lo = b * span;
+    sl_hist(labels, lo, lo + span < n ? lo + span : n, nclusters, h);
+    __syncthreads();
+    if ((int)threadIdx.x <= nclusters) gfb_publish(ctl + SEG_CTL_WORDS, tiles, (int)threadIdx.x, b, h[threadIdx.x]);
+}
+
+__global__ __launch_bounds__(SW_THREADS) void sl_sweep_k(const int32_t* __restrict__ labels, int64_t n,
+                                                         int32_t nclusters, int64_t span, int64_t tiles,
+                                                         uint32_t* __restrict__ ctl, bool counted,
+                                                         int32_t* __restrict__ perm, int64_t* __restrict__ offsets,
+                                                         uint32_t* enc_stats) {
+    __shared__ uint32_t cnt[SW_WAVES][256];
+    __shared__ uint32_t h[256], pre[256], tot[256], base[256], run[256];
+    __shared__ unsigned long long wsum[4];
+    __shared__ uint32_t tile_sh, fail_sh, last_sh;
+    uint32_t* status = ctl + SEG_CTL_WORDS;
+    const int t = threadIdx.x, w = wave_id(), l = lane_id();
+    const int nbins = nclusters + 1;
+    if (t == 0) { tile_sh = atomicAdd(&ctl[0], 1u); fail_sh = 0u; }
+    if (t < 256) { h[t] = 0u; pre[t] = 0u; tot[t] = 0u; }
+    __syncthreads();
+    const int64_t b = tile_sh;
+    const int64_t lo = b * span, hi = lo + span < n ? lo + span : n;
+    if (counted) {
+        sl_hist(labels, lo, hi, nclusters, h);
+        __syncthreads();
+        if (t < nbins) gfb_publish(status, tiles, t, b, h[t]);
+        if (t < nclusters) tot[t] = enc_stats[8 * (int64_t)t + 6];
+    }
+    for (int d0 = w; d0 < nbins; d0 += SW_WAVES * SW_NB) {
+        uint32_t e[SW_NB], a[SW_NB];
+        if (!gfb_sums<SW_NB>(status, tiles, d0, SW_WAVES, nbins, b, counted ? b : tiles, e, a)) {
+            if (l == 0) fail_sh = 1u;
+            break;
+        }
+        if (l == 0) {
+#pragma unroll
+            for (int q = 0; q < SW_NB; ++q) {
+                const int d = d0 + q * SW_WAVES;
+                if (d < nbins) { pre[d] = e[q]; if (!counted) tot[d] = a[q]; }
+            }
+        }
+    }
+    __syncthreads();
+    unsigned long long v = 0, incl = 0;
+    if (t < 256) {
+        v = t < nclusters ? tot[t] : 0u;
+        incl = wave_scan_incl(v);
+        if (l == 63) wsum[w] = incl;
+    }
+    __syncthreads();
+    if (t < 256) {
+        unsigned long long off = 0, sum = 0;
+#pragma unroll
+        for (int w2 = 0; w2 < 4; ++w2) { if (w2 < w) off += wsum[w2]; sum += wsum[w2]; }
+        if (t == 0 && sum > (unsigned long long)n) fail_sh = 1u;
+        base[t] = sum > (unsigned long long)n ? 0u : (uint32_t)(off + incl - v);
+        if (t == nclusters) tot[t] = sum > (unsigned long long)n ? 0u : (uint32_t)((unsigned long long)n - sum);
+        run[t] = base[t] + pre[t];
+    }
+    __syncthreads();
+    if (fail_sh == 0u) {
+        int32_t nx[SW_ROUNDS];
+#pragma unroll
+        for (int r = 0; r < SW_ROUNDS; ++r) {
+            const int64_t i = lo + (int64_t)w * (64 * SW_ROUNDS) + r * 64 + l;
+            nx[r] = i < hi ? labels[i] : -1;
+        }
+        for (int64_t sb = lo; sb < hi; sb += SW_SUB) {
+            for (int j = t; j < SW_WAVES * 256; j += SW_THREADS) (&cnt[0][0])[j] = 0u;
+            __syncthreads();
+            const int64_t seg = sb + (int64_t)w * (64 * SW_ROUNDS);
+            uint32_t bin[SW_ROUNDS], rank[SW_ROUNDS];
+#pragma unroll
+            for (int r = 0; r < SW_ROUNDS; ++r) {
+                bin[r] = sl_bin(nx[r], nclusters);
+                const int64_t i = seg + SW_SUB + r * 64 + l;
+                nx[r] = i < hi ? labels[i] : -1;
+            }
+#pragma unroll
+            for (int r = 0; r < SW_ROUNDS; ++r) {
+                const bool valid = seg + r * 64 + l < hi;
+                const uint32_t d = bin[r];
+                uint32_t peers;
+                const uint32_t rk = wave_match<8>(d, valid, peers);
+                const uint32_t prior = cnt[w][d];
+                __builtin_amdgcn_wave_barrier();
+                if (valid && rk == 0) cnt[w][d] = prior + peers;
+                __builtin_amdgcn_wave_barrier();
+                rank[r] = prior + rk;
+            }
+            __syncthreads();
+            if (t < nbins) {
+                uint32_t at = run[t];
+#pragma unroll
+                for (int w2 = 0; w2 < SW_WAVES; ++w2) {
+                    const uint32_t c = cnt[w2][t];
+                    cnt[w2][t] = at;
+                    at += c;
+                }
+                run[t] = at;
+            }
+            __syncthreads();
+#pragma unroll
+            for (int r = 0; r < SW_ROUNDS; ++r) {
+                const int64_t i = seg + r * 64 + l;
+                const uint32_t pos = cnt[w][bin[r]] + rank[r];
+                if (i < hi && (int64_t)pos < n) perm[pos] = (int32_t)i;
+            }
+            __syncthreads();
+        }
+        if (b == tiles - 1 && t < nbins && run[t] - base[t] != tot[t]) fail_sh = 1u;
+    }
+    __syncthreads();
+    if (t == 0) {
+        if (fail_sh != 0u) atomicOr(&ctl[2], 1u);
+        __threadfence();
+        last_sh = __hip_atomic_fetch_add(&ctl[1], 1u, __ATOMIC_ACQ_REL, __HIP_MEMORY_SCOPE_AGENT) == (uint32_t)(tiles - 1);
+    }
+    __syncthreads();
+    if (last_sh == 0u) return;
+    __threadfence();
+    const bool failed = __hip_atomic_load(&ctl[2], __ATOMIC_RELAXED, __HIP_MEMORY_SCOPE_AGENT) != 0u;
+    if (t < nbins) offsets[t] = failed ? int64_t(-1) : (int64_t)base[t];
+    if (enc_stats)
+        for (int64_t i = t; i < 8 * (int64_t)nclusters; i += SW_THREADS) sg_decode_word(enc_stats, i);
 }
 
 __global__ __launch_bounds__(SG_THREADS) void sg_stats_out_k(const uint32_t* __restrict__ acc, int32_t nclusters,
@@ -226,18 +306,16 @@
 struct SgWs {
     uint64_t *k0, *k1;
     uint32_t *v0, *v1, *radix_ws, *acc;
-    uint32_t *table, *table_scan;
+    uint32_t *sweep;
 };
 static void sg_plan(Arena& a, int64_t n, int32_t nclusters, SgWs& w) {
     const int64_t nn = n > 0 ? n : 1;
     w.acc = a.take<uint32_t>(6 * (size_t)(nclusters > 0 ? nclusters : 1));
     if (nclusters < 256) {
-        const int64_t table = ((int64_t)nclusters + 1) * ceil_div(nn, SL_TILE);
-        w.table = a.take<uint32_t>(table);
-        w.table_scan = a.take<uint32_t>(scan1_pays(table) ? scan1_ws_u32(table) : scan_ws_u32(table));
+        w.sweep = a.take<uint32_t>(SEG_SWEEP_WORDS);
         w.k0 = w.k1 = nullptr; w.v0 = w.v1 = w.radix_ws = nullptr;
     } else {
-        w.table = w.table_scan = nullptr;
+        w.sweep = nullptr;
         w.k0 = a.take<uint64_t>(nn);
         w.k1 = a.take<uint64_t>(nn);
         w.v0 = a.take<uint32_t>(nn);
@@ -268,7 +346,7 @@
 
 int pch::segment_run(const int32_t* labels, const float* xyz, int64_t n, int32_t nclusters, int32_t* out_perm,
                      int64_t* out_offsets, float* out_stats, void* ws, size_t ws_bytes, hipStream_t s,
-                     bool stats_encoded) {
+                     bool stats_encoded, uint32_t* counted_sweep) {
     PCH_REQUIRE(n >= 0 && n < (int64_t(1) << 31) && nclusters >= 0, "bad size");
     PCH_REQUIRE(out_offsets != nullptr, "out_offsets is null");
     if (n == 0) {
@@ -277,28 +355,22 @@
     }
     PCH_REQUIRE(labels && out_perm && ws, "null buffer");
     PCH_REQUIRE(!out_stats || xyz, "stats requested without coordinates");
+    PCH_REQUIRE(!counted_sweep || (stats_encoded && out_stats), "cluster sizes without the encoded table");
     Arena a(ws, ws_bytes);
     SgWs w;
     sg_plan(a, n, nclusters, w);
     if (a.overflow) { set_error("workspace too small: need %zu bytes", a.off); return PCH_ERR_WORKSPACE; }
     const unsigned gn = (unsigned)ceil_div(n, SG_THREADS);
     if (nclusters < 256) {
-        const int64_t nb = ceil_div(n, SL_TILE);
-        const int64_t table = ((int64_t)nclusters + 1) * nb;
-        const bool one = scan1_pays(table);
-        const int64_t zero_words = one ? (int64_t)scan1_ws_u32(table) : 0;
-        PCH_REQUIRE(zero_words <= nb * SG_THREADS, "count table too large for the fused zeroing");
-        PCH_LAUNCH("seg_hist", sl_hist_k, dim3((unsigned)nb), dim3(SG_THREADS), 0, s, labels, n, nclusters,
-                   w.table, nb, w.table_scan, zero_words);
-        const uint32_t* scan_total = one ? w.table_scan + 2 * ceil_div(table, (int64_t)SCAN_TILE) + 1 : nullptr;
-        if (one) PCH_TRY(scan1_exclusive_u32(w.table, w.table, table, w.table_scan, const_cast<uint32_t*>(scan_total), s));
-        else PCH_TRY(scan_exclusive_u32(w.table, w.table, table, w.table_scan, nullptr, s));
-        PCH_LAUNCH("seg_scatter", sl_scatter_k, dim3((unsigned)nb), dim3(SG_THREADS), 0, s, labels, n, nclusters,
-                   (const uint32_t*)w.table, nb, out_perm);
-        PCH_LAUNCH("seg_offsets", sl_offsets_k,
-                   dim3((unsigned)ceil_div(stats_encoded ? 8 * (int64_t)nclusters + 1 : (int64_t)nclusters + 1, SG_THREADS)),
-                   dim3(SG_THREADS), 0, s, (const uint32_t*)w.table, nb, nclusters, out_offsets,
-                   stats_encoded ? reinterpret_cast<uint32_t*>(out_stats) : (uint32_t*)nullptr, scan_total);
+        const SwPlan p = sw_plan(n);
+        const bool counted = counted_sweep != nullptr;
+        uint32_t* ctl = counted ? counted_sweep : w.sweep;
+        if (!counted)
+            PCH_LAUNCH("seg_count", sl_count_k, dim3((unsigned)p.tiles), dim3(SW_THREADS), 0, s, labels, n, nclusters,
+                       p.span, p.tiles, ctl);
+        PCH_LAUNCH("seg_sweep", sl_sweep_k, dim3((unsigned)p.tiles), dim3(SW_THREADS), 0, s, labels, n, nclusters,
+                   p.span, p.tiles, ctl, counted, out_perm, out_offsets,
+                   stats_encoded ? reinterpret_cast<uint32_t*>(out_stats) : (uint32_t*)nullptr);
     } else {
         PCH_LAUNCH("seg_keys", sg_keys_k, dim3(gn), dim3(SG_THREADS), 0, s, labels, n, nclusters, w.k0, w.v0);
         const int nbits = bits_for((uint64_t)nclusters + 1);
diff --git a/profiles/summarize.py b/profiles/summarize.py
--- a/profiles/summarize.py
+++ b/profiles/summarize.py
@@ -51,6 +51,7 @@
          "db_cells_k": "db_cells", "ms_sample_k": "mean_sample", "ms_prefix_k": "mean_prefix",
          "scan1_k<false>": "scan1", "scan1_k<true>": "scan1_popc", "db_prelabel_k": "db_prelabel",
          "sl_hist_k": "seg_hist", "sl_scatter_k": "seg_scatter", "sl_offsets_k": "seg_offsets",
+         "sl_count_k": "seg_count", "sl_sweep_k": "seg_sweep",
          "vx_finish_k": "voxel_finish", "vx_scatter_k": "voxel_scatter", "vx_scatter_lds_k": "voxel_scatter",
          "vx_tilehist_k": "voxel_tilehist", "vx_minmax_k": "voxel_minmax", "vx_split_k": "voxel_split",
          "vx_binscan_k": "voxel_binscan"}
```

New measurement: 60330. 1.4% lower.
